# AsyncFlow-Sim/AsyncFlow

Measured on NVIDIA H100. Metric: simulated request-completions/sec, higher is better.
Workload: dtype f64

## Files before the change

asyncflow_b200/_capi.py:

```python

from __future__ import annotations

import ctypes as C
from pathlib import Path

AF_ABI_VERSION = 1
AF_HIST_BINS = 4096
AF_HIST_SUB_BITS = 7
AF_HIST_MIN_EXP = -20

DIST = {"poisson": 0, "normal": 1, "log_normal": 2, "exponential": 3, "uniform": 4}
TARGET_CLIENT, TARGET_LB, TARGET_SERVER = 0, 1, 2
STEP_CPU, STEP_IO = 0, 1
LB_NONE, LB_ROUND_ROBIN, LB_LEAST_CONNECTIONS = -1, 0, 1
METRIC_BITS = {"ready_queue_len": 1, "event_loop_io_sleep": 2, "ram_in_use": 4,
               "edge_concurrent_connection": 8}
FIELDS = {
    "users_mean": 0, "users_sigma": 1, "rate_per_user": 2, "edge_mean": 3, "edge_sigma": 4,
    "edge_dropout": 5, "server_cpu_cores": 6, "server_ram_mb": 7, "step_duration": 8,
    "endpoint_ram": 9, "spike_delta": 10,
}
FLAG_EVENT_OVERFLOW, FLAG_REQUEST_OVERFLOW, FLAG_TRACE_TRUNCATED, FLAG_NOWQ_OVERFLOW, FLAG_LB_EMPTY = 1, 2, 4, 8, 16
MODE_AUTO, MODE_WARP, MODE_LANE, MODE_TWO_PASS = 0, 1, 2, 3
SELFTEST_EDGE, SELFTEST_GEN_UNIFORM, SELFTEST_GEN_USERS, SELFTEST_ENDPOINT = 0, 1, 2, 3
MODES = {"auto": MODE_AUTO, "warp": MODE_WARP, "lane": MODE_LANE, "two_pass": MODE_TWO_PASS}


class AfEdge(C.Structure):
    _fields_ = [("mean", C.c_double), ("sigma", C.c_double), ("dropout", C.c_double),
                ("dist", C.c_int32), ("target_kind", C.c_int32), ("target_index", C.c_int32),
                ("reserved", C.c_int32)]


class AfServer(C.Structure):
    _fields_ = [("cpu_cores", C.c_int32), ("ram_mb", C.c_int32), ("out_edge", C.c_int32),
                ("endpoint_begin", C.c_int32), ("n_endpoints", C.c_int32), ("reserved", C.c_int32)]


class AfEndpoint(C.Structure):
    _fields_ = [("step_begin", C.c_int32), ("n_steps", C.c_int32), ("total_ram", C.c_int32),
                ("reserved", C.c_int32)]


class AfStep(C.Structure):
    _fields_ = [("duration", C.c_double), ("kind", C.c_int32), ("reserved", C.c_int32)]


class AfSpikeMark(C.Structure):
    _fields_ = [("fire_time", C.c_double), ("delta", C.c_double), ("edge", C.c_int32),
                ("reserved", C.c_int32)]


class AfOutageMark(C.Structure):
    _fields_ = [("fire_time", C.c_double), ("lb_edge", C.c_int32), ("down", C.c_int32)]


class AfScenario(C.Structure):
    _fields_ = [
        ("users_dist", C.c_int32), ("window_s", C.c_int32),
        ("users_mean", C.c_double), ("users_sigma", C.c_double), ("rate_per_user", C.c_double),
        ("horizon_s", C.c_int32), ("metrics_mask", C.c_uint32), ("sample_period", C.c_double),
        ("n_edges", C.c_int32), ("n_servers", C.c_int32), ("n_endpoints", C.c_int32),
        ("n_steps", C.c_int32), ("n_lb_edges", C.c_int32), ("lb_algo", C.c_int32),
        ("gen_edge", C.c_int32), ("client_edge", C.c_int32),
        ("n_spike_marks", C.c_int32), ("n_outage_marks", C.c_int32),
        ("edges", C.POINTER(AfEdge)), ("servers", C.POINTER(AfServer)),
        ("endpoints", C.POINTER(AfEndpoint)), ("steps", C.POINTER(AfStep)),
        ("lb_edges", C.POINTER(C.c_int32)), ("spike_marks", C.POINTER(AfSpikeMark)),
        ("outage_marks", C.POINTER(AfOutageMark)),
    ]


class AfSweepColumn(C.Structure):
    _fields_ = [("field", C.c_int32), ("index", C.c_int32)]


class AfSweep(C.Structure):
    _fields_ = [("n_columns", C.c_int32), ("reserved", C.c_int32), ("n_rows", C.c_uint64),
                ("columns", C.POINTER(AfSweepColumn)), ("values", C.POINTER(C.c_double))]


class AfOptions(C.Structure):
    _fields_ = [("event_capacity", C.c_int32), ("request_capacity", C.c_int32),
                ("warps_per_block", C.c_int32), ("blocks_per_sm", C.c_int32),
                ("collect_histogram", C.c_int32), ("collect_throughput", C.c_int32),
                ("trace_replicas", C.c_int32), ("trace_clock_capacity", C.c_int32)]


class AfReplicaStats(C.Structure):
    _fields_ = [("n_events", C.c_uint64), ("generated", C.c_uint32), ("completed", C.c_uint32),
                ("flags", C.c_uint32), ("n_ticks", C.c_uint32), ("peak_events", C.c_uint32),
                ("peak_requests", C.c_uint32), ("lat_sum", C.c_double), ("lat_sumsq", C.c_double),
                ("lat_min", C.c_double), ("lat_max", C.c_double), ("p50", C.c_double),
                ("p95", C.c_double), ("p99", C.c_double)]


import numpy as np

STATS_DTYPE = np.dtype([
    ("n_events", "<u8"), ("generated", "<u4"), ("completed", "<u4"), ("flags", "<u4"),
    ("n_ticks", "<u4"), ("peak_events", "<u4"), ("peak_requests", "<u4"),
    ("lat_sum", "<f8"), ("lat_sumsq", "<f8"), ("lat_min", "<f8"), ("lat_max", "<f8"),
    ("p50", "<f8"), ("p95", "<f8"), ("p99", "<f8"),
], align=True)
assert STATS_DTYPE.itemsize == C.sizeof(AfReplicaStats)


class AfRunPasses(C.Structure):
    _fields_ = [("lane_pass", C.c_int32), ("warp_pass", C.c_int32), ("lane_warps_per_sm", C.c_int32),
                ("lane_bytes", C.c_int32), ("lane_events_smem", C.c_int32), ("lane_requests_smem", C.c_int32),
                ("lane_replicas", C.c_uint64), ("warp_replicas", C.c_uint64)]


class EngineUnavailable(RuntimeError):
    """The CUDA engine cannot run here (library not built or no usable GPU)."""


LIB_PATH = Path(__file__).resolve().parent / "_lib" / "libasyncflow_b200.so"

EXPORTS = [
    "af_abi_version", "af_engine_create", "af_engine_destroy", "af_last_error",
    "af_engine_configure", "af_scenario_upload", "af_sweep_upload", "af_run", "af_sync",
    "af_last_run_ms", "af_launch_count", "af_fetch_stats", "af_fetch_edge_counts",
    "af_fetch_histograms", "af_fetch_throughput", "af_fetch_sampled", "af_fetch_trace_clocks",
    "af_fetch_trace_series", "af_reduce_histograms", "af_engine_set_mode", "af_last_run_passes",
    "af_selftest_rng",
]

_lib = None


def load() -> C.CDLL:
    global _lib
    if _lib is not None:
        return _lib
    import os
    path = Path(os.environ.get("ASYNCFLOW_B200_LIB", LIB_PATH))
    if not path.exists():
        msg = (f"{path} is missing: build it with `python -c 'import __graft_entry__ as g; "
               "g.build()'` (nvcc, sm_90a).  asyncflow_b200 has no CPU fallback.")
        raise EngineUnavailable(msg)
    lib = C.CDLL(str(path))
    vp, u64, i32 = C.c_void_p, C.c_uint64, C.c_int
    lib.af_abi_version.restype = i32
    lib.af_engine_create.argtypes = [i32, C.POINTER(vp)]
    lib.af_engine_destroy.argtypes = [vp]
    lib.af_engine_destroy.restype = None
    lib.af_last_error.argtypes = [vp]
    lib.af_last_error.restype = C.c_char_p
    lib.af_engine_configure.argtypes = [vp, C.POINTER(AfOptions)]
    lib.af_scenario_upload.argtypes = [vp, C.POINTER(AfScenario)]
    lib.af_sweep_upload.argtypes = [vp, C.POINTER(AfSweep), u64]
    lib.af_run.argtypes = [vp, u64, u64, u64]
    lib.af_sync.argtypes = [vp]
    lib.af_last_run_ms.argtypes = [vp, C.POINTER(C.c_float), C.POINTER(C.c_float)]
    lib.af_launch_count.argtypes = [vp]
    lib.af_launch_count.restype = u64
    lib.af_fetch_stats.argtypes = [vp, vp, u64]
    lib.af_fetch_edge_counts.argtypes = [vp, vp, vp, u64]
    lib.af_fetch_histograms.argtypes = [vp, vp, u64]
    lib.af_fetch_throughput.argtypes = [vp, vp, u64]
    lib.af_fetch_sampled.argtypes = [vp, vp, vp, u64]
    lib.af_fetch_trace_clocks.argtypes = [vp, u64, vp, u64, C.POINTER(u64)]
    lib.af_fetch_trace_series.argtypes = [vp, u64, vp, u64, C.POINTER(u64)]
    lib.af_reduce_histograms.argtypes = [vp, vp]
    lib.af_engine_set_mode.argtypes = [vp, i32]
    lib.af_last_run_passes.argtypes = [vp, C.POINTER(AfRunPasses)]
    lib.af_selftest_rng.argtypes = [vp, u64, u64, i32, i32, C.c_double, C.c_double, C.c_uint32, u64, vp, vp]
    for name in EXPORTS:
        fn = getattr(lib, name)
        if fn.restype is C.c_int and name not in ("af_abi_version",):
            fn.restype = i32
    if lib.af_abi_version() != AF_ABI_VERSION:
        msg = f"ABI mismatch: library {lib.af_abi_version()} != python {AF_ABI_VERSION}"
        raise EngineUnavailable(msg)
    _lib = lib
    return lib
```

asyncflow_b200/csrc/af_engine.cu:

```cuda
#include <cuda_runtime.h>
#include <stdio.h>
#include <stdlib.h>
#include <string.h>
#include <mutex>
#include <new>
#include <string>
#include <vector>

#include "af_host_common.h"
#include "af_lane_host.h"

#ifndef AF_LANE_DEFAULT_WARPS
#define AF_LANE_DEFAULT_WARPS 12
#endif

#ifndef AF_MIN_BLOCKS
#define AF_MIN_BLOCKS 8
#endif
#if AF_MIN_BLOCKS > 0
#define AF_LAUNCH_BOUNDS __launch_bounds__(128, AF_MIN_BLOCKS)
#else
#define AF_LAUNCH_BOUNDS
#endif

__global__ void AF_LAUNCH_BOUNDS af_sim_kernel() {
    extern __shared__ __align__(16) unsigned char af_smem[];
    const int warp = (int)(threadIdx.x >> 5);
    const int lane = (int)(threadIdx.x & 31u);
    unsigned char* ws = af_smem + (size_t)warp * (size_t)afc::c_L.warp_bytes;
    const uint64_t warp_slot = (uint64_t)blockIdx.x * (blockDim.x >> 5) + (uint64_t)warp;
    afc::State& W = *reinterpret_cast<afc::State*>(ws);
    afc::bind(W, ws, warp_slot);
    __syncwarp();
    for (;;) {
        unsigned long long r = 0;
        if (lane == 0) r = atomicAdd(afc::c_G.work_counter, 1ull);
        r = __shfl_sync(0xFFFFFFFFu, r, 0);
        if (afc::c_G.redo_list) {
            if (r >= (unsigned long long)*afc::c_G.redo_count) break;
            r = afc::c_G.redo_list[r];
        } else if (r >= afc::c_G.n_replicas) break;
        afc::run_replica(W, (uint64_t)r);
        __syncwarp();
    }
}

#ifndef AF_LANE_MAX_THREADS
#define AF_LANE_MAX_THREADS 384
#endif
__global__ void __launch_bounds__(AF_LANE_MAX_THREADS, 1) af_lane_kernel() {
    const afl::Cfg& C = afl::c_cfg;
    const uint32_t warp = threadIdx.x >> 5, lane = threadIdx.x & 31u;
    const uint32_t ws = warp * (uint32_t)C.warp_bytes;
    unsigned char* gs = C.gtier + ((uint64_t)blockIdx.x * (blockDim.x >> 5) + warp) * C.gwarp_bytes;
    afl::Mem m;
    m.s128 = ws + lane * 16u;
    m.s64 = ws + (uint32_t)C.n128 * (uint32_t)afl::STRIDE128 + lane * 8u;
    m.s32 = ws + (uint32_t)C.n128 * (uint32_t)afl::STRIDE128 + (uint32_t)C.n64 * (uint32_t)afl::STRIDE64 + lane * 4u;
    m.g128 = gs + lane * 16u;
    m.g64 = gs + (size_t)C.gn128 * afl::STRIDE128 + lane * 8u;
    m.g32 = gs + (size_t)C.gn128 * afl::STRIDE128 + (size_t)C.gn64 * afl::STRIDE64 + lane * 4u;
    afl::run_lane(m,
        [&]() -> uint64_t {
            const unsigned long long k = atomicAdd(C.work_counter, 1ull);
            return k < C.n_replicas ? (uint64_t)k : ~0ull;
        },
        [](bool alive) -> bool { return __any_sync(0xFFFFFFFFu, alive) != 0; });
}

__global__ void af_flagged_kernel(const AfReplicaStats* __restrict__ stats, uint64_t n, uint32_t mask,
                                  uint32_t* __restrict__ list, uint32_t* __restrict__ count) {
    const uint64_t i = (uint64_t)blockIdx.x * blockDim.x + threadIdx.x;
    if (i < n && (stats[i].flags & mask)) list[atomicAdd(count, 1u)] = (uint32_t)i;
}

__global__ void af_selftest_rng_kernel(uint64_t seed, uint64_t replica, int kind, int dist, double mean, double sigma,
                                       uint32_t hop, uint64_t n, double* __restrict__ a, double* __restrict__ b) {
    const uint64_t i = (uint64_t)blockIdx.x * blockDim.x + threadIdx.x;
    if (i >= n) return;
    if (kind == AF_SELFTEST_EDGE) {
        const afr::EdgeDraw d = afr::edge_draw(seed, replica, (uint32_t)i + 1u, hop, dist, mean, sigma, 0.0);
        a[i] = d.u; b[i] = d.transit;
    } else if (kind == AF_SELFTEST_GEN_UNIFORM) {
        afr::Src s = afr::make_gen(seed, replica, (uint32_t)i);
        double u = s.next53();
        a[i] = u;
        if (u < 1e-15) u = 1e-15;
        b[i] = -afr::af_log(1.0 - u);
    } else if (kind == AF_SELFTEST_GEN_USERS) {
        const afr::GenDraw g = afr::gen_users(seed, replica + i, 0u, dist, mean, sigma);
        a[i] = g.value; b[i] = (double)g.pos;
    } else {
        afr::Src src = afr::make_request(seed, replica, afr::P_SERVER, (uint32_t)i + 1u, hop);
        src.load(0);
        a[i] = (double)(uint32_t)(((uint64_t)src.w.x * (uint32_t)dist) >> 32); b[i] = 0.0;
    }
}

__device__ __forceinline__ double af_bin_value(int bin, uint64_t rank, uint64_t cum_before, uint32_t cnt) {
    const long long base = (long long)((1023 + AF_HIST_MIN_EXP) << AF_HIST_SUB_BITS);
    double lo = __longlong_as_double(((long long)bin + base) << (52 - AF_HIST_SUB_BITS));
    double hi = __longlong_as_double(((long long)bin + 1 + base) << (52 - AF_HIST_SUB_BITS));
    double frac = ((double)(rank - cum_before) + 0.5) / (double)cnt;
    return lo + frac * (hi - lo);
}

__global__ void af_percentile_kernel(const uint32_t* __restrict__ hist, AfReplicaStats* __restrict__ stats,
                                     uint64_t n_replicas) {
    const uint64_t warp = ((uint64_t)blockIdx.x * blockDim.x + threadIdx.x) >> 5;
    const int lane = (int)(threadIdx.x & 31u);
    if (warp >= n_replicas) return;
    const uint32_t* row = hist + warp * AF_HIST_BINS;
    const uint64_t n = stats[warp].completed;
    const double qs[3] = {50.0, 95.0, 99.0};
    uint64_t rank[6]; double frac[3]; double val[6];
#pragma unroll
    for (int i = 0; i < 3; ++i) {
        double pos = n ? qs[i] / 100.0 * (double)(n - 1) : 0.0;
        uint64_t lo = (uint64_t)floor(pos);
        frac[i] = pos - (double)lo;
        rank[2 * i] = lo;
        rank[2 * i + 1] = (lo + 1 < n) ? lo + 1 : lo;
        val[2 * i] = val[2 * i + 1] = 0.0;
    }
    uint64_t carry = 0;
    for (int base = 0; base < AF_HIST_BINS; base += 32) {
        uint32_t c = row[base + lane];
        uint32_t incl = c;
#pragma unroll
        for (int d = 1; d < 32; d <<= 1) {
            uint32_t up = __shfl_up_sync(0xFFFFFFFFu, incl, d);
            if (lane >= d) incl += up;
        }
        uint64_t before = carry + (incl - c);
#pragma unroll
        for (int i = 0; i < 6; ++i)
            if (c && rank[i] >= before && rank[i] < before + c) val[i] = af_bin_value(base + lane, rank[i], before, c);
        carry += __shfl_sync(0xFFFFFFFFu, incl, 31);
    }
#pragma unroll
    for (int i = 0; i < 6; ++i) {
        double v = val[i];
#pragma unroll
        for (int d = 16; d > 0; d >>= 1) v += __shfl_xor_sync(0xFFFFFFFFu, v, d);
        val[i] = v;
    }
    if (lane == 0) {
        const double nan = __longlong_as_double(0x7FF8000000000000ll);
        double p[3];
#pragma unroll
        for (int i = 0; i < 3; ++i)
            p[i] = n ? ((frac[i] == 0.0 || rank[2 * i + 1] == rank[2 * i]) ? val[2 * i]
                                                                            : val[2 * i] + frac[i] * (val[2 * i + 1] - val[2 * i]))
                     : nan;
        stats[warp].p50 = p[0]; stats[warp].p95 = p[1]; stats[warp].p99 = p[2];
    }
}


__global__ void af_hist_reduce_kernel(const uint32_t* __restrict__ hist, unsigned long long* __restrict__ total,
                                      uint64_t n_replicas, uint64_t rows_per_block) {
    uint64_t r0 = (uint64_t)blockIdx.x * rows_per_block;
    uint64_t r1 = r0 + rows_per_block < n_replicas ? r0 + rows_per_block : n_replicas;
    unsigned long long acc[AF_HIST_BINS / 256];
#pragma unroll
    for (int j = 0; j < AF_HIST_BINS / 256; ++j) acc[j] = 0;
    for (uint64_t r = r0; r < r1; ++r) {
        const uint32_t* row = hist + r * AF_HIST_BINS;
#pragma unroll
        for (int j = 0; j < AF_HIST_BINS / 256; ++j) acc[j] += row[j * 256 + threadIdx.x];
    }
#pragma unroll
    for (int j = 0; j < AF_HIST_BINS / 256; ++j)
        if (acc[j]) atomicAdd(&total[j * 256 + threadIdx.x], acc[j]);
}

namespace {

struct DevBuf {
    void* p = nullptr; size_t cap = 0;
    cudaError_t ensure(size_t bytes) {
        if (bytes <= cap) return cudaSuccess;
        if (p) cudaFree(p);
        p = nullptr; cap = 0;
        cudaError_t e = cudaMalloc(&p, bytes ? bytes : 1);
        if (e == cudaSuccess) cap = bytes;
        return e;
    }
    void release() { if (p) cudaFree(p); p = nullptr; cap = 0; }
};

thread_local std::string g_create_error;

constexpr int kMaxDevices = 64;
std::mutex g_const_mutex;
af_engine* g_const_owner[kMaxDevices] = {};

}

struct af_engine {
    int device = 0;
    int sm_count = 0;
    int max_smem_optin = 0;
    cudaStream_t stream = nullptr;
    cudaEvent_t ev_begin = nullptr, ev_sim = nullptr, ev_end = nullptr;
    std::string err;
    AfOptions opt{};
    bool have_scenario = false;
    AfScenario sc{};
    std::vector<AfEdge> h_edges; std::vector<AfServer> h_servers; std::vector<AfEndpoint> h_eps;
    std::vector<AfStep> h_steps; std::vector<int32_t> h_lb; std::vector<AfSpikeMark> h_spikes;
    std::vector<AfOutageMark> h_outages;
    DevBuf d_edges, d_servers, d_eps, d_steps, d_lb, d_spikes, d_outages;
    int32_t sweep_cols = 0; uint64_t sweep_rows = 0, sweep_first = 0;
    std::vector<AfSweepColumn> h_sweep_cols;
    std::vector<int32_t> h_sweep_alias;
    int32_t ev_need = 0;
    DevBuf d_sweep_cols, d_sweep_vals;
    int mode = AF_MODE_AUTO;
    aflh::Tables lt;
    DevBuf d_l_edges, d_l_servers, d_l_eps, d_l_steps, d_l_spikes, d_l_outages, d_l_lb, d_l_cols, d_gtier, d_redo_list, d_redo_count, d_counter2;
    afl::Cfg C_host{};
    bool last_lane = false, last_warp = false; int last_lane_warps = 0;
    DevBuf d_sp_evt, d_sp_evk, d_sp_rq, d_sp_nx;
    DevBuf d_stats, d_sent, d_dropped, d_hist, d_thr, d_ssum, d_smax, d_tclk, d_tser, d_tcnt, d_counter, d_htot;
    uint64_t last_n = 0; bool ran = false;
    afc::Layout L{};
    afc::Globals G_host{};
    uint64_t launches = 0;
    float ms_total = 0.f, ms_sim = 0.f; bool timing_valid = false;

    int fail(int code, const std::string& m) { err = m; return code; }
    int cuda_fail(cudaError_t e, const char* what) {
        err = std::string(what) + ": " + cudaGetErrorString(e);
        return AF_ERR_CUDA;
    }
};

#define AF_CUDA(e_, call, what) do { cudaError_t _c = (call); if (_c != cudaSuccess) return (e_)->cuda_fail(_c, what); } while (0)

template <class T>
static int upload_vec(af_engine* e, DevBuf& d, const std::vector<T>& h, const char* what) {
    AF_CUDA(e, d.ensure(h.size() * sizeof(T)), what);
    if (!h.empty()) AF_CUDA(e, cudaMemcpyAsync(d.p, h.data(), h.size() * sizeof(T), cudaMemcpyHostToDevice, e->stream), what);
    return AF_OK;
}

extern "C" {

int af_abi_version(void) { return AF_ABI_VERSION; }

const char* af_last_error(const af_engine* e) { return e ? e->err.c_str() : g_create_error.c_str(); }

int af_engine_create(int device, af_engine** out) {
    if (!out) { g_create_error = "out is NULL"; return AF_ERR_INVALID; }
    *out = nullptr;
    int n = 0;
    cudaError_t ce = cudaGetDeviceCount(&n);
    if (ce != cudaSuccess || n == 0) {
        g_create_error = std::string("no CUDA device: ") + (ce != cudaSuccess ? cudaGetErrorString(ce) : "count is 0")
                         + " (asyncflow_b200 has no CPU fallback)";
        return AF_ERR_CUDA;
    }
    if (device < 0 || device >= n) { g_create_error = "device index out of range"; return AF_ERR_INVALID; }
    cudaDeviceProp prop;
    if ((ce = cudaGetDeviceProperties(&prop, device)) != cudaSuccess) { g_create_error = cudaGetErrorString(ce); return AF_ERR_CUDA; }
    if (prop.major != 9 || prop.minor != 0) {
        char b[160]; snprintf(b, sizeof b, "device %d is sm_%d%d; this library carries sm_90a code only", device, prop.major, prop.minor);
        g_create_error = b; return AF_ERR_CUDA;
    }
    af_engine* e = new (std::nothrow) af_engine();
    if (!e) { g_create_error = "host allocation failed"; return AF_ERR_NOMEM; }
    e->device = device; e->sm_count = prop.multiProcessorCount; e->max_smem_optin = (int)prop.sharedMemPerBlockOptin;
    if ((ce = cudaSetDevice(device)) != cudaSuccess || (ce = cudaStreamCreateWithFlags(&e->stream, cudaStreamNonBlocking)) != cudaSuccess
        || (ce = cudaEventCreate(&e->ev_begin)) != cudaSuccess || (ce = cudaEventCreate(&e->ev_sim)) != cudaSuccess
        || (ce = cudaEventCreate(&e->ev_end)) != cudaSuccess) {
        g_create_error = cudaGetErrorString(ce); delete e; return AF_ERR_CUDA;
    }
    e->opt.collect_histogram = 1; e->opt.collect_throughput = 1;
    if (const char* m = getenv("ASYNCFLOW_B200_ENGINE")) {
        if (!strcmp(m, "warp")) e->mode = AF_MODE_WARP; else if (!strcmp(m, "lane")) e->mode = AF_MODE_LANE;
        else if (!strcmp(m, "two_pass")) e->mode = AF_MODE_TWO_PASS;
    }
    *out = e;
    return AF_OK;
}

void af_engine_destroy(af_engine* e) {
    if (!e) return;
    cudaSetDevice(e->device);
    cudaStreamSynchronize(e->stream);
    {
        std::lock_guard<std::mutex> lock(g_const_mutex);
        if (g_const_owner[e->device % kMaxDevices] == e) g_const_owner[e->device % kMaxDevices] = nullptr;
    }
    DevBuf* bufs[] = {&e->d_l_edges, &e->d_l_servers, &e->d_l_eps, &e->d_l_steps, &e->d_l_spikes, &e->d_l_outages, &e->d_l_lb, &e->d_l_cols,
                      &e->d_gtier, &e->d_redo_list, &e->d_redo_count, &e->d_counter2,
                      &e->d_edges, &e->d_servers, &e->d_eps, &e->d_steps, &e->d_lb, &e->d_spikes, &e->d_outages,
                      &e->d_sweep_cols, &e->d_sweep_vals, &e->d_sp_evt, &e->d_sp_evk, &e->d_sp_rq, &e->d_sp_nx,
                      &e->d_stats, &e->d_sent, &e->d_dropped, &e->d_hist, &e->d_thr, &e->d_ssum, &e->d_smax,
                      &e->d_tclk, &e->d_tser, &e->d_tcnt, &e->d_counter, &e->d_htot};
    for (DevBuf* b : bufs) b->release();
    cudaEventDestroy(e->ev_begin); cudaEventDestroy(e->ev_sim); cudaEventDestroy(e->ev_end);
    cudaStreamDestroy(e->stream);
    delete e;
}

int af_engine_configure(af_engine* e, const AfOptions* opt) {
    if (!e || !opt) return AF_ERR_INVALID;
    if (opt->event_capacity < 0 || opt->request_capacity < 0 || opt->warps_per_block < 0 || opt->warps_per_block > 32 || opt->blocks_per_sm < 0
        || opt->trace_replicas < 0 || opt->trace_clock_capacity < 0)
        return e->fail(AF_ERR_INVALID, "AfOptions: negative or out-of-range field");
    e->opt = *opt;
    return AF_OK;
}

int af_scenario_upload(af_engine* e, const AfScenario* s) {
    if (!e || !s) return AF_ERR_INVALID;
    std::string why;
    if (!afh::validate(*s, why)) return e->fail(AF_ERR_INVALID, "scenario: " + why);
    AF_CUDA(e, cudaSetDevice(e->device), "cudaSetDevice");
    AF_CUDA(e, cudaStreamSynchronize(e->stream), "sync before upload");
    e->sc = *s;
    e->h_edges.assign(s->edges, s->edges + s->n_edges);
    e->h_servers.assign(s->servers, s->servers + s->n_servers);
    e->h_eps.assign(s->endpoints, s->endpoints + s->n_endpoints);
    e->h_steps.assign(s->steps, s->steps + s->n_steps);
    e->h_lb.assign(s->lb_edges, s->lb_edges + s->n_lb_edges);
    e->h_spikes.assign(s->spike_marks, s->spike_marks + s->n_spike_marks);
    e->h_outages.assign(s->outage_marks, s->outage_marks + s->n_outage_marks);
    int rc;
    if ((rc = upload_vec(e, e->d_edges, e->h_edges, "edges"))) return rc;
    if ((rc = upload_vec(e, e->d_servers, e->h_servers, "servers"))) return rc;
    if ((rc = upload_vec(e, e->d_eps, e->h_eps, "endpoints"))) return rc;
    if ((rc = upload_vec(e, e->d_steps, e->h_steps, "steps"))) return rc;
    if ((rc = upload_vec(e, e->d_lb, e->h_lb, "lb_edges"))) return rc;
    if ((rc = upload_vec(e, e->d_spikes, e->h_spikes, "spike_marks"))) return rc;
    if ((rc = upload_vec(e, e->d_outages, e->h_outages, "outage_marks"))) return rc;
    AF_CUDA(e, cudaStreamSynchronize(e->stream), "scenario upload");
    e->sc.edges = e->h_edges.data(); e->sc.servers = e->h_servers.data(); e->sc.endpoints = e->h_eps.data();
    e->sc.steps = e->h_steps.data(); e->sc.lb_edges = e->h_lb.data(); e->sc.spike_marks = e->h_spikes.data();
    e->sc.outage_marks = e->h_outages.data();
    e->have_scenario = true;
    e->sweep_cols = 0; e->sweep_rows = 0; e->h_sweep_cols.clear();
    e->ev_need = aflh::pending_events_estimate(e->sc, nullptr);
    e->ran = false;
    return AF_OK;
}

int af_sweep_upload(af_engine* e, const AfSweep* sw, uint64_t first_replica) {
    if (!e) return AF_ERR_INVALID;
    if (!e->have_scenario) return e->fail(AF_ERR_STATE, "af_sweep_upload before af_scenario_upload");
    AF_CUDA(e, cudaSetDevice(e->device), "cudaSetDevice");
    AF_CUDA(e, cudaStreamSynchronize(e->stream), "sync before sweep upload");
    if (!sw || sw->n_columns == 0 || sw->n_rows == 0) { e->sweep_cols = 0; e->sweep_rows = 0; e->h_sweep_cols.clear(); e->ev_need = aflh::pending_events_estimate(e->sc, nullptr); return AF_OK; }
    if (!sw->columns || !sw->values) return e->fail(AF_ERR_INVALID, "sweep: null columns/values");
    const AfScenario& s = e->sc;
    for (int c = 0; c < sw->n_columns; ++c) {
        int f = sw->columns[c].field, i = sw->columns[c].index, lim = 1;
        switch (f) {
        case AF_FIELD_USERS_MEAN: case AF_FIELD_USERS_SIGMA: case AF_FIELD_RATE_PER_USER: lim = 1; break;
        case AF_FIELD_EDGE_MEAN: case AF_FIELD_EDGE_SIGMA: case AF_FIELD_EDGE_DROPOUT: lim = s.n_edges; break;
        case AF_FIELD_SERVER_CPU_CORES: case AF_FIELD_SERVER_RAM_MB: lim = s.n_servers; break;
        case AF_FIELD_STEP_DURATION: lim = s.n_steps; break;
        case AF_FIELD_ENDPOINT_RAM: lim = s.n_endpoints; break;
        case AF_FIELD_SPIKE_DELTA: lim = s.n_spike_marks; break;
        default: return e->fail(AF_ERR_INVALID, "sweep: unknown field id");
        }
        if (i < 0 || i >= lim) return e->fail(AF_ERR_INVALID, "sweep: column index out of range");
    }
    for (uint64_t r = 0; r < sw->n_rows; ++r)
        for (int c = 0; c < sw->n_columns; ++c) {
            const double v = sw->values[r * (uint64_t)sw->n_columns + (uint64_t)c];
            bool ok = v == v && v - v == 0.0;
            switch (sw->columns[c].field) {
            case AF_FIELD_EDGE_DROPOUT: ok = ok && v >= 0.0 && v <= 1.0; break;
            case AF_FIELD_SERVER_CPU_CORES: case AF_FIELD_SERVER_RAM_MB: ok = ok && v >= 1.0 && v <= 2147483647.0; break;
            case AF_FIELD_ENDPOINT_RAM: ok = ok && v >= 0.0 && v <= 2147483647.0; break;
            case AF_FIELD_EDGE_MEAN: ok = ok && (v >= 0.0 || s.edges[sw->columns[c].index].dist == AF_DIST_LOG_NORMAL || s.edges[sw->columns[c].index].dist == AF_DIST_NORMAL); break;
            case AF_FIELD_USERS_SIGMA: ok = ok && v >= 0.0 && s.users_dist == AF_DIST_NORMAL; break;
            default: ok = ok && v >= 0.0; break;
            }
            if (!ok) {
                char b[200]; snprintf(b, sizeof b, "sweep: row %llu column %d (field %d, index %d): value %g out of range",
                                      (unsigned long long)r, c, sw->columns[c].field, sw->columns[c].index, v);
                return e->fail(AF_ERR_INVALID, b);
            }
        }
    e->h_sweep_cols.assign(sw->columns, sw->columns + sw->n_columns);
    e->h_sweep_alias = aflh::column_aliases(sw->values, sw->n_rows, sw->n_columns);
    e->ev_need = aflh::pending_events_estimate(e->sc, sw);
    size_t cb = (size_t)sw->n_columns * sizeof(AfSweepColumn), vb = (size_t)sw->n_columns * sw->n_rows * sizeof(double);
    AF_CUDA(e, e->d_sweep_cols.ensure(cb), "sweep columns");
    AF_CUDA(e, e->d_sweep_vals.ensure(vb), "sweep values");
    AF_CUDA(e, cudaMemcpyAsync(e->d_sweep_cols.p, sw->columns, cb, cudaMemcpyHostToDevice, e->stream), "sweep columns H2D");
    AF_CUDA(e, cudaMemcpyAsync(e->d_sweep_vals.p, sw->values, vb, cudaMemcpyHostToDevice, e->stream), "sweep values H2D");
    AF_CUDA(e, cudaStreamSynchronize(e->stream), "sweep upload");
    e->sweep_cols = sw->n_columns; e->sweep_rows = sw->n_rows; e->sweep_first = first_replica;
    return AF_OK;
}

static int32_t lane_budget(const af_engine* e, int warps) {
    int32_t b = (int32_t)((e->max_smem_optin / (warps * 32)) & ~3);
    if (const char* cap = getenv("ASYNCFLOW_B200_LANE_BYTES")) { const int32_t c = atoi(cap) & ~3; if (c > 0 && c < b) b = c; }
    return b;
}

int af_run(af_engine* e, uint64_t seed, uint64_t begin, uint64_t end) {
    if (!e) return AF_ERR_INVALID;
    if (!e->have_scenario) return e->fail(AF_ERR_STATE, "af_run before af_scenario_upload");
    if (end <= begin) return e->fail(AF_ERR_INVALID, "af_run: empty replica range");
    if (end - begin > 0xFFFFFFFFull) return e->fail(AF_ERR_INVALID, "af_run: more than 2^32 replicas in one call");
    AF_CUDA(e, cudaSetDevice(e->device), "cudaSetDevice");
    const uint64_t n = end - begin;
    int rc;

    bool lane = e->mode != AF_MODE_WARP;
    afl::Cfg& C = e->C_host;
    int lane_warps = 0;
    if (lane) {
        std::string why;
        const bool all_rows = e->sweep_cols > 0 && begin >= e->sweep_first && end - e->sweep_first <= e->sweep_rows;
        if (!aflh::build_tables(e->sc, e->h_sweep_cols.data(), e->sweep_cols, all_rows ? e->h_sweep_alias.data() : nullptr, e->lt, why)) {
            if (e->mode == AF_MODE_LANE) return e->fail(AF_ERR_INVALID, why);
            lane = false;
        }
    }
    AfOptions o = e->opt;
    if (lane) {
        if (e->mode == AF_MODE_AUTO || e->mode == AF_MODE_TWO_PASS) {
            if (o.event_capacity <= 0 || o.event_capacity > aflh::LANE_EVENT_CAPACITY) o.event_capacity = aflh::LANE_EVENT_CAPACITY;
            if (o.request_capacity <= 0 || o.request_capacity > aflh::LANE_REQUEST_CAPACITY) o.request_capacity = aflh::LANE_REQUEST_CAPACITY;
        }
        lane_warps = e->opt.warps_per_block > 0 ? e->opt.warps_per_block : AF_LANE_DEFAULT_WARPS;
        if (lane_warps > AF_LANE_MAX_THREADS / 32) lane_warps = AF_LANE_MAX_THREADS / 32;
        while (lane_warps > 1 && lane_budget(e, lane_warps) < aflh::min_lane_bytes(e->sc, e->lt) + 128)
            lane_warps -= lane_warps > 8 ? 4 : (lane_warps > 4 ? 2 : 1);
        if (e->mode == AF_MODE_AUTO && lane_warps < 4) lane = false;
        if (e->mode == AF_MODE_AUTO && n < 3ull * (uint64_t)e->sm_count * 32ull) lane = false;
        if (lane && e->opt.warps_per_block <= 0) {
            const uint64_t per_warp = (uint64_t)e->sm_count * 32ull;
            const uint64_t waves = (n + per_warp * (uint64_t)lane_warps - 1) / (per_warp * (uint64_t)lane_warps);
            int w = (int)((n + waves * per_warp - 1) / (waves * per_warp));
            if (w < 4) w = 4;
            if (w < lane_warps) lane_warps = w;
        }
    }
    if (lane) {
        memset(&C, 0, sizeof C);
        if (!aflh::make_cfg(e->sc, o, e->lt, lane_budget(e, lane_warps), afh::trace_tick_capacity(e->sc), 32, C, getenv("ASYNCFLOW_B200_EVEN_SPLIT") ? 0 : e->ev_need,
                            getenv("ASYNCFLOW_B200_RQ_MIN") ? atoi(getenv("ASYNCFLOW_B200_RQ_MIN")) : 2)) {
            if (e->mode == AF_MODE_LANE) return e->fail(AF_ERR_INVALID, "scenario tables do not fit a lane's shared memory (thread-per-replica engine)");
            lane = false;
        }
    }
    const bool warp = e->mode != AF_MODE_LANE;
    const bool redo = lane && warp;

    afc::Layout& L = e->L;
    memset(&L, 0, sizeof L);
    afh::make_layout(e->sc, e->opt, e->sweep_cols, L);

    int wpb = 4; size_t smem = 0; uint64_t grid = 0, warp_slots = 0;
    if (warp) {
        if (!lane && e->opt.warps_per_block > 0 && e->opt.warps_per_block < 4) wpb = e->opt.warps_per_block;
        smem = (size_t)wpb * (size_t)L.warp_bytes;
        while (wpb > 1 && smem > (size_t)e->max_smem_optin) { --wpb; smem = (size_t)wpb * (size_t)L.warp_bytes; }
        if (smem > (size_t)e->max_smem_optin)
            return e->fail(AF_ERR_INVALID, "scenario tables do not fit in shared memory (one warp needs more than the 227 KB opt-in limit)");
        AF_CUDA(e, cudaFuncSetAttribute(af_sim_kernel, cudaFuncAttributeMaxDynamicSharedMemorySize, (int)smem), "smem attribute");
        int bps = 0;
        AF_CUDA(e, cudaOccupancyMaxActiveBlocksPerMultiprocessor(&bps, af_sim_kernel, wpb * 32, smem), "occupancy");
        if (bps < 1) return e->fail(AF_ERR_CUDA, "kernel cannot be resident (occupancy 0)");
        if (e->opt.blocks_per_sm > 0 && e->opt.blocks_per_sm < bps) bps = e->opt.blocks_per_sm;
        grid = (uint64_t)e->sm_count * (uint64_t)bps;
        const uint64_t need_blocks = (n + wpb - 1) / wpb;
        if (grid > need_blocks) grid = need_blocks;
        warp_slots = grid * wpb;
    }
    uint64_t lgrid = 0; size_t lsmem = 0;
    if (lane) {
        lsmem = (size_t)lane_warps * (size_t)C.warp_bytes;
        AF_CUDA(e, cudaFuncSetAttribute(af_lane_kernel, cudaFuncAttributeMaxDynamicSharedMemorySize, (int)lsmem), "smem attribute");
        lgrid = (uint64_t)e->sm_count;
        const uint64_t need = (n + (uint64_t)lane_warps * 32 - 1) / ((uint64_t)lane_warps * 32);
        if (lgrid > need) lgrid = need;
    }

    if (warp) {
        const uint64_t ev_sp = (uint64_t)(L.ev_total - L.ev_smem), rq_sp = (uint64_t)(L.rq_total - L.rq_smem);
        AF_CUDA(e, e->d_sp_evt.ensure(warp_slots * ev_sp * 8 + 8), "spill events");
        AF_CUDA(e, e->d_sp_evk.ensure(warp_slots * ev_sp * 8 + 8), "spill events");
        AF_CUDA(e, e->d_sp_rq.ensure(warp_slots * rq_sp * 16 + 16), "spill requests");
        AF_CUDA(e, e->d_sp_nx.ensure(warp_slots * rq_sp * 4 + 4), "spill requests");
    }
    if (lane) {
        AF_CUDA(e, e->d_gtier.ensure(lgrid * (uint64_t)lane_warps * C.gwarp_bytes + 256), "lane global tiers");
        if ((rc = upload_vec(e, e->d_l_edges, e->lt.edges, "lane tables"))) return rc;
        if ((rc = upload_vec(e, e->d_l_servers, e->lt.servers, "lane tables"))) return rc;
        if ((rc = upload_vec(e, e->d_l_eps, e->lt.endpoints, "lane tables"))) return rc;
        if ((rc = upload_vec(e, e->d_l_steps, e->lt.steps, "lane tables"))) return rc;
        if ((rc = upload_vec(e, e->d_l_spikes, e->lt.spikes, "lane tables"))) return rc;
        if ((rc = upload_vec(e, e->d_l_outages, e->lt.outages, "lane tables"))) return rc;
        if ((rc = upload_vec(e, e->d_l_lb, e->lt.lb, "lane tables"))) return rc;
        if ((rc = upload_vec(e, e->d_l_cols, e->lt.cols, "lane tables"))) return rc;
        AF_CUDA(e, e->d_counter2.ensure(8), "work counter");
        AF_CUDA(e, e->d_redo_list.ensure(n * 4), "flagged-replica list");
        AF_CUDA(e, e->d_redo_count.ensure(4), "flagged-replica count");
    }
    const uint64_t ntr = (uint64_t)(L.trace_replicas < 0 ? 0 : L.trace_replicas) < n ? (uint64_t)L.trace_replicas : n;
    L.trace_replicas = (int32_t)ntr; C.trace_replicas = (int32_t)ntr;
    AF_CUDA(e, e->d_stats.ensure(n * sizeof(AfReplicaStats)), "stats");
    AF_CUDA(e, e->d_sent.ensure(n * L.n_edges * 4), "edge counts");
    AF_CUDA(e, e->d_dropped.ensure(n * L.n_edges * 4), "edge counts");
    AF_CUDA(e, e->d_ssum.ensure(n * L.n_series * 8), "sampled sums");
    AF_CUDA(e, e->d_smax.ensure(n * L.n_series * 4), "sampled maxima");
    AF_CUDA(e, e->d_counter.ensure(8), "work counter");
    if (L.collect_hist) AF_CUDA(e, e->d_hist.ensure(n * AF_HIST_BINS * 4), "histograms");
    if (L.collect_thr) AF_CUDA(e, e->d_thr.ensure(n * (uint64_t)L.horizon_s * 4), "throughput");
    if (ntr) {
        AF_CUDA(e, e->d_tclk.ensure(ntr * (uint64_t)L.trace_clock_cap * 16 + 16), "trace clocks");
        AF_CUDA(e, e->d_tser.ensure(ntr * (uint64_t)L.n_series * (uint64_t)L.trace_tick_cap * 4 + 4), "trace series");
    }
    AF_CUDA(e, e->d_tcnt.ensure((ntr ? ntr : 1) * 8), "trace counts");

    afc::Globals G;
    memset(&G, 0, sizeof G);
    G.edges = (const AfEdge*)e->d_edges.p; G.servers = (const AfServer*)e->d_servers.p;
    G.endpoints = (const AfEndpoint*)e->d_eps.p; G.steps = (const AfStep*)e->d_steps.p;
    G.lb_edges = (const int32_t*)e->d_lb.p; G.spikes = (const AfSpikeMark*)e->d_spikes.p;
    G.outages = (const AfOutageMark*)e->d_outages.p;
    G.sweep_cols = (const AfSweepColumn*)e->d_sweep_cols.p; G.sweep_vals = (const double*)e->d_sweep_vals.p;
    G.sweep_first = e->sweep_first; G.sweep_rows = e->sweep_cols ? e->sweep_rows : 0;
    G.spill_ev_time = (double*)e->d_sp_evt.p; G.spill_ev_key = (uint64_t*)e->d_sp_evk.p;
    G.spill_rq_rec = (afc::ReqRec*)e->d_sp_rq.p; G.spill_rq_next = (uint32_t*)e->d_sp_nx.p;
    G.stats = (AfReplicaStats*)e->d_stats.p; G.edge_sent = (uint32_t*)e->d_sent.p; G.edge_dropped = (uint32_t*)e->d_dropped.p;
    G.hist = (uint32_t*)e->d_hist.p; G.thr = (uint32_t*)e->d_thr.p;
    G.samp_sum = (uint64_t*)e->d_ssum.p; G.samp_max = (uint32_t*)e->d_smax.p;
    G.trace_clocks = (double*)e->d_tclk.p; G.trace_series = (uint32_t*)e->d_tser.p; G.trace_counts = (uint32_t*)e->d_tcnt.p;
    G.work_counter = (unsigned long long*)e->d_counter.p;
    G.redo_list = redo ? (const uint32_t*)e->d_redo_list.p : nullptr;
    G.redo_count = redo ? (const uint32_t*)e->d_redo_count.p : nullptr;
    G.seed = seed; G.replica_begin = begin; G.n_replicas = n;
    if (lane) {
        C.edges = (const afl::EdgeP*)e->d_l_edges.p; C.servers = (const afl::ServerP*)e->d_l_servers.p;
        C.endpoints = (const afl::EndpointP*)e->d_l_eps.p; C.steps = (const afl::StepP*)e->d_l_steps.p;
        C.spikes = (const afl::SpikeP*)e->d_l_spikes.p; C.outages = (const afl::OutageP*)e->d_l_outages.p;
        C.lb_edges = (const int32_t*)e->d_l_lb.p; C.cols = (const afl::ColP*)e->d_l_cols.p;
        C.sweep_vals = G.sweep_vals; C.sweep_first = G.sweep_first; C.sweep_rows = G.sweep_rows;
        C.gtier = (unsigned char*)e->d_gtier.p;
        C.stats = G.stats; C.edge_sent = G.edge_sent; C.edge_dropped = G.edge_dropped; C.hist = G.hist; C.thr = G.thr;
        C.samp_sum = G.samp_sum; C.samp_max = G.samp_max; C.trace_clocks = G.trace_clocks; C.trace_series = G.trace_series;
        C.trace_counts = G.trace_counts;
        C.work_counter = (unsigned long long*)e->d_counter2.p;
        C.seed = seed; C.replica_begin = begin; C.n_replicas = n;
    }

    std::lock_guard<std::mutex> lock(g_const_mutex);
    {
        af_engine*& owner = g_const_owner[e->device % kMaxDevices];
        if (owner && owner != e) AF_CUDA(e, cudaStreamSynchronize(owner->stream), "waiting for the device's previous engine");
        owner = e;
    }
    AF_CUDA(e, cudaEventRecord(e->ev_begin, e->stream), "event");
    AF_CUDA(e, cudaMemsetAsync(e->d_counter.p, 0, 8, e->stream), "memset");
    if (L.collect_hist) AF_CUDA(e, cudaMemsetAsync(e->d_hist.p, 0, n * AF_HIST_BINS * 4, e->stream), "memset hist");
    if (L.collect_thr) AF_CUDA(e, cudaMemsetAsync(e->d_thr.p, 0, n * (uint64_t)L.horizon_s * 4, e->stream), "memset thr");
    if (lane) {
        AF_CUDA(e, cudaMemsetAsync(e->d_counter2.p, 0, 8, e->stream), "memset");
        AF_CUDA(e, cudaMemsetAsync(e->d_redo_count.p, 0, 4, e->stream), "memset");
        AF_CUDA(e, cudaMemcpyToSymbolAsync(afl::c_cfg, &C, sizeof C, 0, cudaMemcpyHostToDevice, e->stream), "lane config -> constant memory");
        af_lane_kernel<<<(unsigned)lgrid, lane_warps * 32, lsmem, e->stream>>>();
        AF_CUDA(e, cudaGetLastError(), "af_lane_kernel launch");
        e->launches += 1;
        if (redo) {
            af_flagged_kernel<<<(unsigned)((n + 255) / 256), 256, 0, e->stream>>>((const AfReplicaStats*)e->d_stats.p, n,
                AF_FLAG_EVENT_OVERFLOW | AF_FLAG_REQUEST_OVERFLOW | AF_FLAG_NOWQ_OVERFLOW, (uint32_t*)e->d_redo_list.p, (uint32_t*)e->d_redo_count.p);
            AF_CUDA(e, cudaGetLastError(), "af_flagged_kernel launch");
            e->launches += 1;
        }
    }
    if (warp) {
        AF_CUDA(e, cudaMemcpyToSymbolAsync(afc::c_L, &L, sizeof L, 0, cudaMemcpyHostToDevice, e->stream), "layout -> constant memory");
        e->G_host = G;
        AF_CUDA(e, cudaMemcpyToSymbolAsync(afc::c_G, &e->G_host, sizeof G, 0, cudaMemcpyHostToDevice, e->stream), "globals -> constant memory");
        af_sim_kernel<<<(unsigned)grid, wpb * 32, smem, e->stream>>>();
        AF_CUDA(e, cudaGetLastError(), "af_sim_kernel launch");
        e->launches += 1;
    }
    AF_CUDA(e, cudaEventRecord(e->ev_sim, e->stream), "event");
    if (L.collect_hist) {
        unsigned blocks = (unsigned)((n * 32 + 255) / 256);
        af_percentile_kernel<<<blocks, 256, 0, e->stream>>>((const uint32_t*)e->d_hist.p, (AfReplicaStats*)e->d_stats.p, n);
        AF_CUDA(e, cudaGetLastError(), "af_percentile_kernel launch");
        e->launches += 1;
    }
    AF_CUDA(e, cudaEventRecord(e->ev_end, e->stream), "event");
    e->last_n = n; e->ran = true; e->timing_valid = false;
    e->last_lane = lane; e->last_warp = warp; e->last_lane_warps = lane_warps;
    return AF_OK;
}

int af_selftest_rng(af_engine* e, uint64_t seed, uint64_t replica, int kind, int dist, double mean, double sigma,
                    uint32_t hop, uint64_t n, double* out_a, double* out_b) {
    if (!e || !out_a || !out_b || n == 0) return AF_ERR_INVALID;
    if (kind < AF_SELFTEST_EDGE || kind > AF_SELFTEST_ENDPOINT) return e->fail(AF_ERR_INVALID, "af_selftest_rng: unknown kind");
    AF_CUDA(e, cudaSetDevice(e->device), "cudaSetDevice");
    DevBuf da, db;
    cudaError_t ce;
    if ((ce = da.ensure(n * 8)) != cudaSuccess || (ce = db.ensure(n * 8)) != cudaSuccess) { da.release(); db.release(); return e->cuda_fail(ce, "selftest buffers"); }
    af_selftest_rng_kernel<<<(unsigned)((n + 255) / 256), 256, 0, e->stream>>>(seed, replica, kind, dist, mean, sigma, hop, n, (double*)da.p, (double*)db.p);
    e->launches += 1;
    ce = cudaGetLastError();
    if (ce == cudaSuccess) ce = cudaMemcpyAsync(out_a, da.p, n * 8, cudaMemcpyDeviceToHost, e->stream);
    if (ce == cudaSuccess) ce = cudaMemcpyAsync(out_b, db.p, n * 8, cudaMemcpyDeviceToHost, e->stream);
    if (ce == cudaSuccess) ce = cudaStreamSynchronize(e->stream);
    da.release(); db.release();
    if (ce != cudaSuccess) return e->cuda_fail(ce, "af_selftest_rng");
    return AF_OK;
}

int af_engine_set_mode(af_engine* e, int mode) {
    if (!e) return AF_ERR_INVALID;
    if (mode != AF_MODE_AUTO && mode != AF_MODE_WARP && mode != AF_MODE_LANE && mode != AF_MODE_TWO_PASS) return e->fail(AF_ERR_INVALID, "af_engine_set_mode: unknown mode");
    e->mode = mode;
    return AF_OK;
}

int af_last_run_passes(af_engine* e, AfRunPasses* out) {
    if (!e || !out) return AF_ERR_INVALID;
    if (!e->ran) return e->fail(AF_ERR_STATE, "no run yet");
    int rc = af_sync(e);
    if (rc) return rc;
    memset(out, 0, sizeof *out);
    out->lane_pass = e->last_lane ? 1 : 0; out->warp_pass = e->last_warp ? 1 : 0;
    out->lane_warps_per_sm = e->last_lane_warps;
    out->lane_bytes = e->last_lane ? e->C_host.warp_bytes / 32 : 0;
    out->lane_events_smem = e->last_lane ? e->C_host.ev_s : 0; out->lane_requests_smem = e->last_lane ? e->C_host.rq_s : 0;
    out->lane_replicas = e->last_lane ? e->last_n : 0;
    out->warp_replicas = e->last_warp ? e->last_n : 0;
    if (e->last_lane && e->last_warp) {
        uint32_t c = 0;
        AF_CUDA(e, cudaMemcpyAsync(&c, e->d_redo_count.p, 4, cudaMemcpyDeviceToHost, e->stream), "flagged count D2H");
        AF_CUDA(e, cudaStreamSynchronize(e->stream), "flagged count D2H");
        out->warp_replicas = c;
    }
    return AF_OK;
}

int af_sync(af_engine* e) {
    if (!e) return AF_ERR_INVALID;
    AF_CUDA(e, cudaSetDevice(e->device), "cudaSetDevice");
    AF_CUDA(e, cudaStreamSynchronize(e->stream), "af_sync");
    if (e->ran && !e->timing_valid) {
        float a = 0.f, b = 0.f;
        if (cudaEventElapsedTime(&a, e->ev_begin, e->ev_end) == cudaSuccess
            && cudaEventElapsedTime(&b, e->ev_begin, e->ev_sim) == cudaSuccess) {
            e->ms_total = a; e->ms_sim = b; e->timing_valid = true;
        }
    }
    return AF_OK;
}

int af_last_run_ms(af_engine* e, float* ms_total, float* ms_sim) {
    if (!e) return AF_ERR_INVALID;
    if (!e->ran) return e->fail(AF_ERR_STATE, "no run yet");
    int rc = af_sync(e);
    if (rc) return rc;
    if (ms_total) *ms_total = e->ms_total;
    if (ms_sim) *ms_sim = e->ms_sim;
    return AF_OK;
}

uint64_t af_launch_count(const af_engine* e) { return e ? e->launches : 0; }

static int fetch(af_engine* e, void* dst, const DevBuf& src, size_t bytes, uint64_t n, const char* what) {
    if (!e || !dst) return AF_ERR_INVALID;
    if (!e->ran) return e->fail(AF_ERR_STATE, "fetch before af_run");
    if (n != e->last_n) return e->fail(AF_ERR_INVALID, "fetch: n differs from the last run's replica count");
    AF_CUDA(e, cudaSetDevice(e->device), "cudaSetDevice");
    AF_CUDA(e, cudaMemcpyAsync(dst, src.p, bytes, cudaMemcpyDeviceToHost, e->stream), what);
    return af_sync(e);
}

int af_fetch_stats(af_engine* e, AfReplicaStats* out, uint64_t n) {
    return fetch(e, out, e->d_stats, n * sizeof(AfReplicaStats), n, "stats D2H");
}
int af_fetch_edge_counts(af_engine* e, uint32_t* sent, uint32_t* dropped, uint64_t n) {
    int rc = fetch(e, sent, e->d_sent, n * e->L.n_edges * 4, n, "edge sent D2H");
    if (rc) return rc;
    return fetch(e, dropped, e->d_dropped, n * e->L.n_edges * 4, n, "edge dropped D2H");
}
int af_fetch_histograms(af_engine* e, uint32_t* out, uint64_t n) {
    if (e && e->ran && !e->L.collect_hist) return e->fail(AF_ERR_STATE, "histograms were not collected");
    return fetch(e, out, e->d_hist, n * AF_HIST_BINS * 4, n, "hist D2H");
}
int af_fetch_throughput(af_engine* e, uint32_t* out, uint64_t n) {
    if (e && e->ran && !e->L.collect_thr) return e->fail(AF_ERR_STATE, "throughput was not collected");
    return fetch(e, out, e->d_thr, n * (uint64_t)e->L.horizon_s * 4, n, "throughput D2H");
}
int af_fetch_sampled(af_engine* e, uint64_t* sums, uint32_t* maxima, uint64_t n) {
    int rc = fetch(e, sums, e->d_ssum, n * e->L.n_series * 8, n, "sampled sums D2H");
    if (rc) return rc;
    return fetch(e, maxima, e->d_smax, n * e->L.n_series * 4, n, "sampled maxima D2H");
}

int af_reduce_histograms(af_engine* e, uint64_t* out_bins) {
    if (!e || !out_bins) return AF_ERR_INVALID;
    if (!e->ran) return e->fail(AF_ERR_STATE, "reduce before af_run");
    if (!e->L.collect_hist) return e->fail(AF_ERR_STATE, "histograms were not collected");
    AF_CUDA(e, cudaSetDevice(e->device), "cudaSetDevice");
    AF_CUDA(e, e->d_htot.ensure(AF_HIST_BINS * 8), "histogram total");
    AF_CUDA(e, cudaMemsetAsync(e->d_htot.p, 0, AF_HIST_BINS * 8, e->stream), "memset");
    const uint64_t n = e->last_n;
    uint64_t blocks = (uint64_t)e->sm_count * 8;
    if (blocks > n) blocks = n;
    uint64_t rows = (n + blocks - 1) / blocks;
    blocks = (n + rows - 1) / rows;
    af_hist_reduce_kernel<<<(unsigned)blocks, 256, 0, e->stream>>>((const uint32_t*)e->d_hist.p,
                                                                  (unsigned long long*)e->d_htot.p, n, rows);
    AF_CUDA(e, cudaGetLastError(), "af_hist_reduce_kernel launch");
    e->launches += 1;
    AF_CUDA(e, cudaMemcpyAsync(out_bins, e->d_htot.p, AF_HIST_BINS * 8, cudaMemcpyDeviceToHost, e->stream), "hist total D2H");
    AF_CUDA(e, cudaStreamSynchronize(e->stream), "af_reduce_histograms");
    return AF_OK;
}

int af_fetch_trace_clocks(af_engine* e, uint64_t local, double* out, uint64_t cap_pairs, uint64_t* n_pairs) {
    if (!e || !out || !n_pairs) return AF_ERR_INVALID;
    if (!e->ran) return e->fail(AF_ERR_STATE, "fetch before af_run");
    if (local >= (uint64_t)e->L.trace_replicas) return e->fail(AF_ERR_INVALID, "replica was not traced");
    AF_CUDA(e, cudaSetDevice(e->device), "cudaSetDevice");
    uint32_t cnt[2];
    AF_CUDA(e, cudaMemcpyAsync(cnt, (uint32_t*)e->d_tcnt.p + local * 2, 8, cudaMemcpyDeviceToHost, e->stream), "trace counts");
    AF_CUDA(e, cudaStreamSynchronize(e->stream), "trace counts");
    uint64_t n = cnt[0];
    if (n > (uint64_t)e->L.trace_clock_cap) n = (uint64_t)e->L.trace_clock_cap;
    if (n > cap_pairs) n = cap_pairs;
    *n_pairs = n;
    if (n) AF_CUDA(e, cudaMemcpyAsync(out, (double*)e->d_tclk.p + local * (uint64_t)e->L.trace_clock_cap * 2, n * 16,
                                      cudaMemcpyDeviceToHost, e->stream), "trace clocks");
    return af_sync(e);
}

int af_fetch_trace_series(af_engine* e, uint64_t local, uint32_t* out, uint64_t cap_ticks, uint64_t* n_ticks) {
    if (!e || !out || !n_ticks) return AF_ERR_INVALID;
    if (!e->ran) return e->fail(AF_ERR_STATE, "fetch before af_run");
    if (local >= (uint64_t)e->L.trace_replicas) return e->fail(AF_ERR_INVALID, "replica was not traced");
    AF_CUDA(e, cudaSetDevice(e->device), "cudaSetDevice");
    uint32_t cnt[2];
    AF_CUDA(e, cudaMemcpyAsync(cnt, (uint32_t*)e->d_tcnt.p + local * 2, 8, cudaMemcpyDeviceToHost, e->stream), "trace counts");
    AF_CUDA(e, cudaStreamSynchronize(e->stream), "trace counts");
    uint64_t n = cnt[1];
    if (n > (uint64_t)e->L.trace_tick_cap) n = (uint64_t)e->L.trace_tick_cap;
    if (n > cap_ticks) n = cap_ticks;
    *n_ticks = n;
    const uint32_t* base = (const uint32_t*)e->d_tser.p + local * (uint64_t)e->L.n_series * (uint64_t)e->L.trace_tick_cap;
    if (n) AF_CUDA(e, cudaMemcpy2DAsync(out, cap_ticks * 4, base, (size_t)e->L.trace_tick_cap * 4, n * 4, (size_t)e->L.n_series,
                                        cudaMemcpyDeviceToHost, e->stream), "trace series");
    return af_sync(e);
}

}
```

asyncflow_b200/csrc/af_lane.cuh:

```cuda
#pragma once
#include "af_rng.cuh"
#include "../../include/asyncflow_b200.h"

#if defined(__CUDA_ARCH__)
#define AFL_DEVICE 1
#else
#define AFL_DEVICE 0
#endif

#if defined(__CUDACC__)
#define AFL_IN __host__ __device__ __forceinline__
#else
#define AFL_IN static inline
#endif

#define AFL_LIKELY(x) __builtin_expect(!!(x), 1)
#define AFL_UNLIKELY(x) __builtin_expect(!!(x), 0)

#if defined(AF_TRACE_HOST) && !AFL_DEVICE
#include <stdio.h>
#define AFL_TRACE(...) fprintf(stderr, __VA_ARGS__)
#else
#define AFL_TRACE(...) ((void)0)
#endif

namespace afl {

#if AFL_DEVICE
constexpr int LANES = 32;
#else
constexpr int LANES = 1;
#endif
constexpr int STRIDE128 = LANES * 16, STRIDE64 = LANES * 8, STRIDE32 = LANES * 4;

constexpr uint32_t NIL = 0xFFFFFFFFu;
constexpr uint64_t INF_BITS = 0x7FF0000000000000ull;

enum : uint32_t { K_ARRIVAL = 0, K_DELIVER = 1, K_STEP_END = 2, K_SPIKE = 3, K_OUTAGE = 4 };
constexpr uint32_t SLOT_BITS = 20, AUX_BITS = 9;
constexpr uint32_t SLOT_MASK = (1u << SLOT_BITS) - 1, AUX_MASK = (1u << AUX_BITS) - 1;
AFL_IN uint32_t mk_payload(uint32_t kind, uint32_t aux, uint32_t slot) { return (kind << 29) | (aux << SLOT_BITS) | slot; }

constexpr uint32_t PK_CORE = 1u << 28, PK_IO = 1u << 29, PK_WAIT = 1u << 30;
AFL_IN uint32_t pk_hops(uint32_t p) { return p & 0xFFu; }
AFL_IN uint32_t pk_step(uint32_t p) { return (p >> 8) & 0xFFu; }
AFL_IN uint32_t pk_ep(uint32_t p) { return (p >> 16) & 0xFFFu; }

enum : uint32_t { I_PUT = 0, I_GOT = 1, I_CLIENT_LOOP = 2, I_RAM_OK = 3, I_CPU_OK = 4, I_CPU_PUT = 5, I_RAM_PUT = 6 };
constexpr uint32_t NODE_CLIENT = 0, NODE_LB = 1, NODE_SERVER0 = 2;
constexpr int32_t NQ_TOTAL = 128;

struct alignas(16) EdgeP { double mean, sigma, dropout; uint32_t meta; int16_t c_mean, c_sigma, c_drop, pad; uint32_t pad2[2]; };
struct alignas(16) ServerP { int32_t cpu_cores, ram_mb; uint32_t out_edge, ep_begin, n_ep; int32_t c_cores, c_ram, pad; };
struct alignas(16) EndpointP { uint32_t step_begin, n_steps, total_ram; int32_t c_ram; };
struct alignas(16) StepP { double dur; uint32_t kind; int32_t c_dur; };
struct alignas(16) SpikeP { double fire, delta; uint32_t edge; int32_t c_delta; uint32_t pad[2]; };
struct alignas(16) OutageP { double fire; int32_t lb_edge, down; };
struct ColP { int32_t field, index, slot, pad; double base; };

enum : int32_t { SV_CPU_FREE = 0, SV_RAM_FREE, SV_READY_Q, SV_IO_Q, SV_RAM_IN_USE, SV_WORDS };
enum : int32_t { SQ_RAMQ_HEAD = 0, SQ_RAMQ_TAIL, SQ_CPUQ_HEAD, SQ_CPUQ_TAIL, SQ_RAMQ_NEED, SQ_WORDS };
enum : int32_t { IB_HEAD = 0, IB_TAIL, IB_PENDING, IB_WORDS };

struct Cfg {
    int32_t n_edges, n_servers, n_endpoints, n_steps, n_lb_edges, lb_algo;
    int32_t gen_edge, client_edge, n_spike, n_outage;
    int32_t users_dist, window_s, horizon_s;
    uint32_t metrics_mask;
    double users_mean, users_sigma, rate_per_user, sample_period;
    int32_t n_series, n_sweep_cols, n_row;
    int32_t collect_hist, collect_thr, trace_replicas, trace_clock_cap, trace_tick_cap;
    int32_t redo;
    int32_t ev_s, ev_total, rq_s, rq_total, nq_s;
    int32_t o128_ev, o128_rq, n128;
    int32_t o64_nq, o64_spike, o64_row, n64;
    int32_t o32_next, o32_conn, o32_srv, o32_lb, o32_dirty, n_dirty, n32;
    int32_t warp_bytes;
    int32_t gi_ev, gi_rq, gn128;
    int32_t gi_nq, gi_acc, gn64;
    int32_t gi_next, g32_cold, gi_smax, gi_sent, gn32;
    int32_t c_srvq, c_inbox, c_drop;
    uint64_t gwarp_bytes;
    const EdgeP* edges; const ServerP* servers; const EndpointP* endpoints; const StepP* steps;
    const SpikeP* spikes; const OutageP* outages; const int32_t* lb_edges; const ColP* cols;
    const double* sweep_vals; uint64_t sweep_first, sweep_rows;
    unsigned char* gtier;
    AfReplicaStats* stats; uint32_t* edge_sent; uint32_t* edge_dropped;
    uint32_t* hist; uint32_t* thr; uint64_t* samp_sum; uint32_t* samp_max;
    double* trace_clocks; uint32_t* trace_series; uint32_t* trace_counts;
    unsigned long long* work_counter;
    const uint32_t* redo_list; const uint32_t* redo_count;
    uint64_t seed, replica_begin, n_replicas;
};

#if defined(__CUDACC__)
__constant__ Cfg c_cfg;
#endif
#if AFL_DEVICE
#define AFL_C c_cfg
#else
static Cfg h_cfg;
#define AFL_C h_cfg
#endif

template <class T> AFL_IN T ro(const T* p) {
#if AFL_DEVICE
    static_assert(sizeof(T) % 16 == 0, "16-byte records");
    T v;
    const uint4* s = reinterpret_cast<const uint4*>(p);
    uint4* d = reinterpret_cast<uint4*>(&v);
#pragma unroll
    for (int i = 0; i < (int)(sizeof(T) / 16); ++i) d[i] = __ldg(s + i);
    return v;
#else
    return *p;
#endif
}

struct Mem {
    uint32_t s128, s64, s32;
    unsigned char* g128; unsigned char* g64; unsigned char* g32;
};
#if AFL_DEVICE
AFL_IN uint32_t sm_ld32(uint32_t a) { uint32_t v; asm volatile("ld.shared.u32 %0, [%1];" : "=r"(v) : "r"(a)); return v; }
AFL_IN void sm_st32(uint32_t a, uint32_t v) { asm volatile("st.shared.u32 [%0], %1;" :: "r"(a), "r"(v)); }
AFL_IN uint64_t sm_ld64(uint32_t a) { uint64_t v; asm volatile("ld.shared.u64 %0, [%1];" : "=l"(v) : "r"(a)); return v; }
AFL_IN void sm_st64(uint32_t a, uint64_t v) { asm volatile("st.shared.u64 [%0], %1;" :: "r"(a), "l"(v)); }
AFL_IN void sm_ld128(uint32_t a, uint64_t& x, uint64_t& y) { asm volatile("ld.shared.v2.u64 {%0, %1}, [%2];" : "=l"(x), "=l"(y) : "r"(a)); }
AFL_IN void sm_st128(uint32_t a, uint64_t x, uint64_t y) { asm volatile("st.shared.v2.u64 [%0], {%1, %2};" :: "r"(a), "l"(x), "l"(y)); }
AFL_IN void gl_ld128(const unsigned char* p, uint64_t& x, uint64_t& y) { const ulonglong2 v = *reinterpret_cast<const ulonglong2*>(p); x = v.x; y = v.y; }
AFL_IN void gl_st128(unsigned char* p, uint64_t x, uint64_t y) { *reinterpret_cast<ulonglong2*>(p) = make_ulonglong2(x, y); }
#else
static unsigned char* afl_smem_host = nullptr;
AFL_IN uint32_t sm_ld32(uint32_t a) { uint32_t v; memcpy(&v, afl_smem_host + a, 4); return v; }
AFL_IN void sm_st32(uint32_t a, uint32_t v) { memcpy(afl_smem_host + a, &v, 4); }
AFL_IN uint64_t sm_ld64(uint32_t a) { uint64_t v; memcpy(&v, afl_smem_host + a, 8); return v; }
AFL_IN void sm_st64(uint32_t a, uint64_t v) { memcpy(afl_smem_host + a, &v, 8); }
AFL_IN void sm_ld128(uint32_t a, uint64_t& x, uint64_t& y) { memcpy(&x, afl_smem_host + a, 8); memcpy(&y, afl_smem_host + a + 8, 8); }
AFL_IN void sm_st128(uint32_t a, uint64_t x, uint64_t y) { memcpy(afl_smem_host + a, &x, 8); memcpy(afl_smem_host + a + 8, &y, 8); }
AFL_IN void gl_ld128(const unsigned char* p, uint64_t& x, uint64_t& y) { memcpy(&x, p, 8); memcpy(&y, p + 8, 8); }
AFL_IN void gl_st128(unsigned char* p, uint64_t x, uint64_t y) { memcpy(p, &x, 8); memcpy(p + 8, &y, 8); }
#endif
AFL_IN uint32_t a128(const Mem& m, int32_t elem) { return m.s128 + (uint32_t)elem * (uint32_t)STRIDE128; }
AFL_IN uint32_t a64(const Mem& m, int32_t elem) { return m.s64 + (uint32_t)elem * (uint32_t)STRIDE64; }
AFL_IN uint32_t a32(const Mem& m, int32_t word) { return m.s32 + (uint32_t)word * (uint32_t)STRIDE32; }
AFL_IN unsigned char* g128p(const Mem& m, int32_t elem) { return m.g128 + (uint64_t)(uint32_t)elem * (uint32_t)STRIDE128; }
AFL_IN uint64_t* g64p(const Mem& m, int32_t elem) { return reinterpret_cast<uint64_t*>(m.g64 + (uint64_t)(uint32_t)elem * (uint32_t)STRIDE64); }
AFL_IN uint32_t* g32p(const Mem& m, int32_t word) { return reinterpret_cast<uint32_t*>(m.g32 + (uint64_t)(uint32_t)word * (uint32_t)STRIDE32); }
AFL_IN uint64_t e64_ld(const Mem& m, int32_t elem) { return sm_ld64(a64(m, elem)); }
AFL_IN void e64_st(const Mem& m, int32_t elem, uint64_t v) { sm_st64(a64(m, elem), v); }
AFL_IN double f64_ld(const Mem& m, int32_t elem) { return afr::u2d(e64_ld(m, elem)); }
AFL_IN void f64_st(const Mem& m, int32_t elem, double v) { e64_st(m, elem, afr::d2u(v)); }
AFL_IN uint32_t w32_ld(const Mem& m, int32_t word) { return sm_ld32(a32(m, word)); }
AFL_IN void w32_st(const Mem& m, int32_t word, uint32_t v) { sm_st32(a32(m, word), v); }
AFL_IN int32_t i32_ld(const Mem& m, int32_t word) { return (int32_t)w32_ld(m, word); }
AFL_IN void i32_st(const Mem& m, int32_t word, int32_t v) { w32_st(m, word, (uint32_t)v); }
AFL_IN uint32_t c32_ld(const Mem& m, int32_t word) { return *g32p(m, AFL_C.g32_cold + word); }
AFL_IN void c32_st(const Mem& m, int32_t word, uint32_t v) { *g32p(m, AFL_C.g32_cold + word) = v; }
AFL_IN void ld_t128(const Mem& m, int32_t os, int32_t gi, int32_t idx, int32_t split, uint64_t& x, uint64_t& y) {
    if (AFL_LIKELY(idx < split)) sm_ld128(a128(m, os + idx), x, y); else gl_ld128(g128p(m, gi + idx), x, y);
}
AFL_IN void st_t128(const Mem& m, int32_t os, int32_t gi, int32_t idx, int32_t split, uint64_t x, uint64_t y) {
    if (AFL_LIKELY(idx < split)) sm_st128(a128(m, os + idx), x, y); else gl_st128(g128p(m, gi + idx), x, y);
}
AFL_IN uint64_t ld_t64(const Mem& m, int32_t os, int32_t gi, int32_t idx, int32_t split) {
    if (AFL_LIKELY(idx < split)) return sm_ld64(a64(m, os + idx));
    return *g64p(m, gi + idx);
}
AFL_IN void st_t64(const Mem& m, int32_t os, int32_t gi, int32_t idx, int32_t split, uint64_t v) {
    if (AFL_LIKELY(idx < split)) sm_st64(a64(m, os + idx), v); else *g64p(m, gi + idx) = v;
}
AFL_IN uint32_t ld_t32(const Mem& m, int32_t os, int32_t gi, int32_t idx, int32_t split) {
    if (AFL_LIKELY(idx < split)) return sm_ld32(a32(m, os + idx));
    return *g32p(m, gi + idx);
}
AFL_IN void st_t32(const Mem& m, int32_t os, int32_t gi, int32_t idx, int32_t split, uint32_t v) {
    if (AFL_LIKELY(idx < split)) sm_st32(a32(m, os + idx), v); else *g32p(m, gi + idx) = v;
}

struct St {
    uint64_t replica, local;
    double now, horizon;
    uint32_t seq; int32_t ev_n; uint32_t peak_ev;
    uint64_t arr_t; uint32_t arr_seq, arr_on;
    uint32_t nq_head, nq_tail, busy;
    uint32_t rq_free, rq_free_hi, rq_hw, rq_live, peak_rq;
    uint32_t n_waiting;
    double g_vnow, g_wend, g_lam;
    uint32_t g_pos, generated, g_done, need_arrival, arm_seq;
    double gap0, gap1; uint32_t gap_cnt;
    double users_mean, users_sigma, rate_per_user;
    int32_t lb_n, spike_cur, outage_cur;
    uint32_t tick_seq, n_ticks; double tick_time;
    uint32_t completed, flags, traced;
    uint64_t n_events;
    double lat_sum, lat_sumsq, lat_min, lat_max;
};

constexpr uint32_t STOP_FLAGS = AF_FLAG_EVENT_OVERFLOW | AF_FLAG_REQUEST_OVERFLOW | AF_FLAG_NOWQ_OVERFLOW | AF_FLAG_LB_EMPTY;

AFL_IN double row_val(const Mem& m, int32_t c) { return f64_ld(m, AFL_C.o64_row + c); }
AFL_IN uint32_t ep_total_ram(const Mem& m, uint32_t ep) {
    const EndpointP p = ro(AFL_C.endpoints + ep);
    return p.c_ram >= 0 ? (uint32_t)row_val(m, p.c_ram) : p.total_ram;
}

AFL_IN void rq_load(const Mem& m, uint32_t s, double& t0, uint32_t& rid, uint32_t& pack) {
    uint64_t a, b;
    ld_t128(m, AFL_C.o128_rq, AFL_C.gi_rq, (int32_t)s, AFL_C.rq_s, a, b);
    t0 = afr::u2d(a); rid = (uint32_t)b; pack = (uint32_t)(b >> 32);
}
AFL_IN void rq_store(const Mem& m, uint32_t s, double t0, uint32_t rid, uint32_t pack) {
    st_t128(m, AFL_C.o128_rq, AFL_C.gi_rq, (int32_t)s, AFL_C.rq_s, afr::d2u(t0), (uint64_t)rid | ((uint64_t)pack << 32));
}
AFL_IN uint32_t rq_pack(const Mem& m, uint32_t s) {
    if (AFL_LIKELY((int32_t)s < AFL_C.rq_s)) return sm_ld32(a128(m, AFL_C.o128_rq + (int32_t)s) + 12u);
    return *reinterpret_cast<const uint32_t*>(g128p(m, AFL_C.gi_rq + (int32_t)s) + 12);
}
AFL_IN void rq_pack_set(const Mem& m, uint32_t s, uint32_t v) {
    if (AFL_LIKELY((int32_t)s < AFL_C.rq_s)) sm_st32(a128(m, AFL_C.o128_rq + (int32_t)s) + 12u, v);
    else *reinterpret_cast<uint32_t*>(g128p(m, AFL_C.gi_rq + (int32_t)s) + 12) = v;
}
AFL_IN uint32_t rq_next(const Mem& m, uint32_t s) { return ld_t32(m, AFL_C.o32_next, AFL_C.gi_next, (int32_t)s, AFL_C.rq_s); }
AFL_IN void rq_next_set(const Mem& m, uint32_t s, uint32_t v) { st_t32(m, AFL_C.o32_next, AFL_C.gi_next, (int32_t)s, AFL_C.rq_s, v); }

#if AFL_DEVICE
__device__ __forceinline__ void red_add64(uint64_t* p, uint64_t v) { atomicAdd(reinterpret_cast<unsigned long long*>(p), (unsigned long long)v); }
__device__ __forceinline__ void red_add32(uint32_t* p, uint32_t v) { atomicAdd(p, v); }
__device__ __forceinline__ void red_max32(uint32_t* p, uint32_t v) { atomicMax(p, v); }
__device__ __forceinline__ uint64_t ld_cg64(const uint64_t* p) { return (uint64_t)__ldcg(reinterpret_cast<const unsigned long long*>(p)); }
__device__ __forceinline__ uint32_t ld_cg32(const uint32_t* p) { return __ldcg(p); }
#else
static inline void red_add64(uint64_t* p, uint64_t v) { *p += v; }
static inline void red_add32(uint32_t* p, uint32_t v) { *p += v; }
static inline void red_max32(uint32_t* p, uint32_t v) { if (v > *p) *p = v; }
static inline uint64_t ld_cg64(const uint64_t* p) { return *p; }
static inline uint32_t ld_cg32(const uint32_t* p) { return *p; }
#endif
AFL_IN uint32_t rq_alloc(St& W, const Mem& m) {
    uint32_t s;
    if (W.rq_free != NIL) { s = W.rq_free; W.rq_free = rq_next(m, s); }
    else if ((int32_t)W.rq_hw < AFL_C.rq_s) { s = W.rq_hw++; }
    else if (W.rq_free_hi != NIL) { s = W.rq_free_hi; W.rq_free_hi = rq_next(m, s); }
    else if ((int32_t)W.rq_hw < AFL_C.rq_total) { s = W.rq_hw++; }
    else { W.flags |= AF_FLAG_REQUEST_OVERFLOW; return NIL; }
    const uint32_t live = ++W.rq_live;
    if (live > W.peak_rq) W.peak_rq = live;
    return s;
}
AFL_IN void rq_release(St& W, const Mem& m, uint32_t s) {
    if ((int32_t)s < AFL_C.rq_s) { rq_next_set(m, s, W.rq_free); W.rq_free = s; }
    else { rq_next_set(m, s, W.rq_free_hi); W.rq_free_hi = s; }
    --W.rq_live;
}

#if defined(__CUDACC__)
#define AFL_COLD __host__ __device__ __noinline__
#else
#define AFL_COLD static __attribute__((noinline))
#endif
AFL_COLD void fifo_push(const Mem m, int32_t w_head, int32_t w_tail, uint32_t s) {
    rq_next_set(m, s, NIL);
    const uint32_t tail = c32_ld(m, w_tail);
    if (tail == NIL) c32_st(m, w_head, s); else rq_next_set(m, tail, s);
    c32_st(m, w_tail, s);
}
AFL_COLD uint32_t fifo_pop(const Mem m, int32_t w_head, int32_t w_tail) {
    const uint32_t s = c32_ld(m, w_head);
    const uint32_t h = rq_next(m, s);
    c32_st(m, w_head, h);
    if (h == NIL) c32_st(m, w_tail, NIL);
    return s;
}

AFL_IN void ev_get(const Mem& m, int32_t i, uint64_t& t, uint64_t& k) { ld_t128(m, AFL_C.o128_ev, AFL_C.gi_ev, i, AFL_C.ev_s, t, k); }
AFL_IN void ev_set(const Mem& m, int32_t i, uint64_t t, uint64_t k) { st_t128(m, AFL_C.o128_ev, AFL_C.gi_ev, i, AFL_C.ev_s, t, k); }
AFL_IN bool ev_less(uint64_t ta, uint64_t ka, uint64_t tb, uint64_t kb) {
    return ta < tb || (ta == tb && (uint32_t)(ka >> 32) < (uint32_t)(kb >> 32));
}
AFL_IN void heap_push(St& W, const Mem& m, uint64_t tb, uint64_t key) {
    int32_t i = W.ev_n;
    const int32_t pending = i + (int32_t)W.arr_on;
    if (AFL_UNLIKELY(pending >= AFL_C.ev_total)) { W.flags |= AF_FLAG_EVENT_OVERFLOW; return; }
    W.ev_n = i + 1;
    if ((uint32_t)(pending + 1) > W.peak_ev) W.peak_ev = (uint32_t)(pending + 1);
#pragma unroll 1
    while (i > 0) {
        const int32_t p = (i - 1) >> 2;
        uint64_t tp, kp;
        ev_get(m, p, tp, kp);
        if (!ev_less(tb, key, tp, kp)) break;
        ev_set(m, i, tp, kp);
        i = p;
    }
    ev_set(m, i, tb, key);
}
AFL_IN void heap_pop(St& W, const Mem& m) {
    const int32_t n = --W.ev_n;
    if (n == 0) return;
    uint64_t tl, kl;
    ev_get(m, n, tl, kl);
    const int32_t last = n - 1;
    int32_t i = 0;
#pragma unroll 1
    for (;;) {
        const int32_t c = 4 * i + 1;
        if (c >= n) break;
        const int32_t c1 = c + 1 < last ? c + 1 : last, c3 = c + 3 < last ? c + 3 : last;
        int32_t c2 = c + 2 < last ? c + 2 : last;
        uint64_t t0, k0, t1, k1, t2, k2, t3, k3;
        if (AFL_LIKELY(c3 < AFL_C.ev_s)) {
            sm_ld128(a128(m, AFL_C.o128_ev + c), t0, k0); sm_ld128(a128(m, AFL_C.o128_ev + c1), t1, k1);
            sm_ld128(a128(m, AFL_C.o128_ev + c2), t2, k2); sm_ld128(a128(m, AFL_C.o128_ev + c3), t3, k3);
        } else {
            ev_get(m, c, t0, k0); ev_get(m, c1, t1, k1); ev_get(m, c2, t2, k2); ev_get(m, c3, t3, k3);
        }
        int32_t b = c;
        if (ev_less(t1, k1, t0, k0)) { t0 = t1; k0 = k1; b = c1; }
        if (ev_less(t3, k3, t2, k2)) { t2 = t3; k2 = k3; c2 = c3; }
        if (ev_less(t2, k2, t0, k0)) { t0 = t2; k0 = k2; b = c2; }
        if (!ev_less(t0, k0, tl, kl)) break;
        ev_set(m, i, t0, k0);
        i = b;
    }
    ev_set(m, i, tl, kl);
}

AFL_IN uint64_t nq_ld(const Mem& m, uint32_t pos) {
    return ld_t64(m, AFL_C.o64_nq, AFL_C.gi_nq, (int32_t)(pos & (uint32_t)(NQ_TOTAL - 1)), AFL_C.nq_s);
}
AFL_IN bool can_fuse(const St& W) { return AFL_LIKELY(W.busy == 0); }
AFL_IN void nq_push(St& W, const Mem& m, uint32_t kind, uint32_t aux, uint32_t slot) {
    const uint32_t tail = W.nq_tail;
    if (tail - W.nq_head >= (uint32_t)NQ_TOTAL) { W.flags |= AF_FLAG_NOWQ_OVERFLOW; return; }
    st_t64(m, AFL_C.o64_nq, AFL_C.gi_nq, (int32_t)(tail & (uint32_t)(NQ_TOTAL - 1)), AFL_C.nq_s,
           ((uint64_t)(W.seq++) << 32) | mk_payload(kind, aux, slot));
    W.nq_tail = tail + 1;
    W.busy += 2u;
}
AFL_IN uint32_t nq_take(St& W, const Mem& m) {
    const uint32_t item = (uint32_t)nq_ld(m, W.nq_head);
    W.nq_head += 1;
    if (W.nq_head == W.nq_tail) { W.nq_head = 0; W.nq_tail = 0; }
    return item;
}

AFL_IN bool gen_next_gap(St& W, double& gap) {
    const double T = W.horizon;
    double vnow = W.g_vnow, wend = W.g_wend, lam = W.g_lam;
    uint32_t pos = W.g_pos;
    bool ok = false;
#pragma unroll 1
    for (;;) {
        if (!(vnow < T)) break;
        if (vnow >= wend) {
            wend = vnow + (double)AFL_C.window_s;
            afr::GenDraw d = afr::gen_users(AFL_C.seed, W.replica, pos, AFL_C.users_dist, W.users_mean, W.users_sigma);
            pos = d.pos;
            lam = d.value * W.rate_per_user;
        }
        if (lam <= 0.0) { vnow = wend; continue; }
        afr::Src s = afr::make_gen(AFL_C.seed, W.replica, pos);
        double u = s.next53();
        pos = s.pos;
        if (u < 1e-15) u = 1e-15;
        const double dt = afr::af_div(-afr::af_log(1.0 - u), lam);
        if (vnow + dt > T) break;
        if (vnow + dt >= wend) { vnow = wend; continue; }
        vnow += dt;
        gap = dt;
        ok = true;
        break;
    }
    W.g_vnow = vnow; W.g_wend = wend; W.g_lam = lam; W.g_pos = pos;
    return ok;
}

AFL_IN void gauge_touch(const St& W, const Mem& m, int32_t j, uint32_t v_old, int32_t delta) {
    red_add64(g64p(m, AFL_C.gi_acc + j), (uint64_t)(int64_t)delta * (uint64_t)W.n_ticks);
    const int32_t dw = AFL_C.o32_dirty + (j >> 5);
    const uint32_t d = w32_ld(m, dw), bit = 1u << (j & 31);
    if (!(d & bit)) {
        red_max32(g32p(m, AFL_C.gi_smax + j), v_old);
        w32_st(m, dw, d | bit);
    }
}
AFL_IN void conn_add(const St& W, const Mem& m, uint32_t edge, int32_t delta) {
    const int32_t pw = AFL_C.o32_conn + (int32_t)edge;
    const uint32_t v = w32_ld(m, pw);
    if (AFL_C.metrics_mask & AF_METRIC_EDGE_CONN) gauge_touch(W, m, 3 * AFL_C.n_servers + (int32_t)edge, v, delta);
    w32_st(m, pw, v + (uint32_t)delta);
}
AFL_IN int32_t ib_word(uint32_t node, int32_t f) { return AFL_C.c_inbox + (int32_t)node * IB_WORDS + f; }
AFL_IN int32_t sq_word(uint32_t sidx, int32_t f) { return AFL_C.c_srvq + (int32_t)sidx * SQ_WORDS + f; }
AFL_IN int32_t sv_word(uint32_t sidx, int32_t f) { return AFL_C.o32_srv + (int32_t)sidx * SV_WORDS + f; }
AFL_IN void srv_gauge_add(const St& W, const Mem& m, uint32_t sidx, int32_t field, int32_t delta) {
    const int32_t pw = sv_word(sidx, field);
    const int32_t v = i32_ld(m, pw);
    if ((AFL_C.metrics_mask & 7u) == 7u) gauge_touch(W, m, 3 * (int32_t)sidx + (field - SV_READY_Q), (uint32_t)v, delta);
    i32_st(m, pw, v + delta);
}
AFL_IN uint32_t gauge_value(const Mem& m, int32_t j) {
    const int32_t ns3 = 3 * AFL_C.n_servers;
    if (j < ns3) { const int32_t mt = j % 3; return w32_ld(m, sv_word((uint32_t)(j / 3), mt == 0 ? SV_READY_Q : (mt == 1 ? SV_IO_Q : SV_RAM_IN_USE))); }
    return w32_ld(m, AFL_C.o32_conn + (j - ns3));
}
AFL_IN bool gauge_on(int32_t j) {
    return j < 3 * AFL_C.n_servers ? (AFL_C.metrics_mask & 7u) == 7u
                                   : (AFL_C.metrics_mask & AF_METRIC_EDGE_CONN) != 0;
}
AFL_IN void take_ticks(St& W, const Mem& m, double t, uint32_t ev_seq) {
    double tick = W.tick_time;
    uint32_t tseq = W.tick_seq, nt = W.n_ticks, seq = W.seq;
    const double horizon = W.horizon;
#pragma unroll 1
    while ((tick < t || (tick == t && tseq < ev_seq)) && tick < horizon) {
        if (AFL_UNLIKELY(W.traced != 0) && (int32_t)nt < AFL_C.trace_tick_cap) {
#pragma unroll 1
            for (int32_t j = 0; j < AFL_C.n_series; ++j)
                if (gauge_on(j)) AFL_C.trace_series[(W.local * (uint64_t)AFL_C.n_series + (uint32_t)j) * (uint64_t)AFL_C.trace_tick_cap + nt] = gauge_value(m, j);
        }
        nt += 1;
        tseq = seq++;
        tick = tick + AFL_C.sample_period;
    }
    if (nt != W.n_ticks) {
#pragma unroll 1
        for (int32_t w = 0; w < AFL_C.n_dirty; ++w) w32_st(m, AFL_C.o32_dirty + w, 0u);
    }
    W.tick_time = tick; W.tick_seq = tseq; W.n_ticks = nt; W.seq = seq;
}

AFL_IN bool q_empty(const St& W, const Mem& m, int32_t head) { return AFL_LIKELY(W.n_waiting == 0) || c32_ld(m, head) == NIL; }
AFL_IN void consumer_get(St& W, const Mem& m, uint32_t node) {
    if (AFL_UNLIKELY(c32_ld(m, ib_word(node, IB_HEAD)) != NIL)) {
        const uint32_t it = fifo_pop(m, ib_word(node, IB_HEAD), ib_word(node, IB_TAIL));
        nq_push(W, m, I_GOT, node, it);
    } else c32_st(m, ib_word(node, IB_PENDING), 1);
}
AFL_IN bool cpu_walk(St& W, const Mem& m, uint32_t sidx, uint32_t watch) {
    bool hit = false;
#pragma unroll 1
    while (!q_empty(W, m, sq_word(sidx, SQ_CPUQ_HEAD)) && i32_ld(m, sv_word(sidx, SV_CPU_FREE)) > 0) {
        const uint32_t w = fifo_pop(m, sq_word(sidx, SQ_CPUQ_HEAD), sq_word(sidx, SQ_CPUQ_TAIL));
        W.n_waiting -= 1;
        i32_st(m, sv_word(sidx, SV_CPU_FREE), i32_ld(m, sv_word(sidx, SV_CPU_FREE)) - 1);
        hit = hit || w == watch;
        nq_push(W, m, I_CPU_OK, sidx, w);
    }
    return hit;
}
AFL_IN void ram_walk(St& W, const Mem& m, uint32_t sidx) {
#pragma unroll 1
    while (!q_empty(W, m, sq_word(sidx, SQ_RAMQ_HEAD))) {
        const uint32_t need = c32_ld(m, sq_word(sidx, SQ_RAMQ_NEED));
        if ((int32_t)need > i32_ld(m, sv_word(sidx, SV_RAM_FREE))) break;
        const uint32_t w = fifo_pop(m, sq_word(sidx, SQ_RAMQ_HEAD), sq_word(sidx, SQ_RAMQ_TAIL));
        W.n_waiting -= 1;
        const uint32_t h = c32_ld(m, sq_word(sidx, SQ_RAMQ_HEAD));
        if (h != NIL) c32_st(m, sq_word(sidx, SQ_RAMQ_NEED), ep_total_ram(m, pk_ep(rq_pack(m, h))));
        i32_st(m, sv_word(sidx, SV_RAM_FREE), i32_ld(m, sv_word(sidx, SV_RAM_FREE)) - (int32_t)need);
        nq_push(W, m, I_RAM_OK, sidx, w);
    }
}

AFL_IN bool on_spike(St& W, const Mem& m, double& next_fire) {
    int32_t cur = W.spike_cur;
    const double t = ro(AFL_C.spikes + cur).fire;
#pragma unroll 1
    while (cur < AFL_C.n_spike) {
        const SpikeP p = ro(AFL_C.spikes + cur);
        if (p.fire != t) break;
        double delta = p.delta;
        if (p.c_delta >= 0) { const double v = row_val(m, p.c_delta); delta = delta < 0.0 ? -v : v; }
        f64_st(m, AFL_C.o64_spike + (int32_t)p.edge, f64_ld(m, AFL_C.o64_spike + (int32_t)p.edge) + delta);
        ++cur;
    }
    W.spike_cur = cur;
    if (cur < AFL_C.n_spike) { next_fire = ro(AFL_C.spikes + cur).fire; return true; }
    return false;
}
AFL_IN bool on_outage(St& W, const Mem& m, double& next_fire) {
    int32_t cur = W.outage_cur;
    const double t = ro(AFL_C.outages + cur).fire;
    int32_t n = W.lb_n;
    const int32_t lb = AFL_C.o32_lb;
#pragma unroll 1
    while (cur < AFL_C.n_outage) {
        const OutageP p = ro(AFL_C.outages + cur);
        if (p.fire != t) break;
        ++cur;
        if (p.lb_edge < 0) continue;
        int32_t at = -1;
#pragma unroll 1
        for (int32_t i = 0; i < n; ++i) if (w32_ld(m, lb + i) == (uint32_t)p.lb_edge) { at = i; break; }
        if (at >= 0) {
#pragma unroll 1
            for (int32_t i = at + 1; i < n; ++i) w32_st(m, lb + i - 1, w32_ld(m, lb + i));
            --n;
        }
        if (!p.down) { w32_st(m, lb + n, (uint32_t)p.lb_edge); ++n; }
    }
    W.lb_n = n;
    W.outage_cur = cur;
    if (cur < AFL_C.n_outage) { next_fire = ro(AFL_C.outages + cur).fire; return true; }
    return false;
}

#if AFL_DEVICE
__device__ __forceinline__ void red_add(uint32_t* p, uint32_t v) { atomicAdd(p, v); }
#else
static inline void red_add(uint32_t* p, uint32_t v) { *p += v; }
#endif

AFL_IN void complete(St& W, const Mem& m, uint32_t slot, double t0) {
    const double now = W.now;
    const double lat = now - t0;
    const uint32_t done = ++W.completed;
    W.lat_sum += lat;
    W.lat_sumsq += lat * lat;
    if (lat < W.lat_min) W.lat_min = lat;
    if (lat > W.lat_max) W.lat_max = lat;
    const uint64_t local = W.local;
    if (AFL_C.collect_hist) {
        int32_t idx = (int32_t)(afr::d2u(lat) >> (52 - AF_HIST_SUB_BITS)) - ((1023 + AF_HIST_MIN_EXP) << AF_HIST_SUB_BITS);
        idx = idx < 0 ? 0 : (idx >= AF_HIST_BINS ? AF_HIST_BINS - 1 : idx);
        red_add(&AFL_C.hist[local * AF_HIST_BINS + (uint32_t)idx], 1u);
    }
    if (AFL_C.collect_thr) {
        int32_t b = (int32_t)ceil(now) - 1;
        b = b < 0 ? 0 : b;
        if (b < AFL_C.horizon_s) red_add(&AFL_C.thr[local * (uint64_t)AFL_C.horizon_s + (uint32_t)b], 1u);
    }
    if (AFL_UNLIKELY(W.traced != 0)) {
        if ((int32_t)(done - 1) < AFL_C.trace_clock_cap) {
            double* p = AFL_C.trace_clocks + (local * (uint64_t)AFL_C.trace_clock_cap + (done - 1)) * 2;
            p[0] = t0; p[1] = now;
        } else W.flags |= AF_FLAG_TRACE_TRUNCATED;
    }
    rq_release(W, m, slot);
}

AFL_IN void start_replica(St& W, const Mem& m, uint64_t local_index) {
    const Cfg& C = AFL_C;
    W.local = local_index;
    W.replica = C.replica_begin + local_index;
    W.now = 0.0; W.horizon = (double)C.horizon_s; W.seq = 0;
    W.ev_n = 0; W.peak_ev = 0; W.arr_t = 0; W.arr_seq = 0; W.arr_on = 0;
    W.nq_head = 0; W.nq_tail = 0; W.busy = 0;
    W.rq_free = NIL; W.rq_free_hi = NIL; W.rq_hw = 0; W.rq_live = 0; W.peak_rq = 0; W.n_waiting = 0;
    W.g_vnow = 0.0; W.g_wend = 0.0; W.g_lam = 0.0; W.g_pos = 0; W.generated = 0; W.g_done = 0;
    W.gap0 = 0.0; W.gap1 = 0.0; W.gap_cnt = 0;
    W.lb_n = C.n_lb_edges; W.spike_cur = 0; W.outage_cur = 0;
    W.n_ticks = 0; W.completed = 0; W.flags = 0; W.n_events = 0;
    W.lat_sum = 0.0; W.lat_sumsq = 0.0; W.lat_min = afr::u2d(INF_BITS); W.lat_max = 0.0;
    W.traced = (int64_t)local_index < (int64_t)C.trace_replicas ? 1u : 0u;
    W.users_mean = C.users_mean; W.users_sigma = C.users_sigma; W.rate_per_user = C.rate_per_user;
#pragma unroll 1
    for (int32_t i = 0; i < C.n_edges; ++i) {
        w32_st(m, C.o32_conn + i, 0); *g32p(m, C.gi_sent + i) = 0; c32_st(m, C.c_drop + i, 0);
        if (C.n_spike > 0) f64_st(m, C.o64_spike + i, 0.0);
    }
#pragma unroll 1
    for (int32_t i = 0; i < C.n_servers; ++i) {
        const ServerP p = ro(C.servers + i);
        i32_st(m, sv_word((uint32_t)i, SV_CPU_FREE), p.cpu_cores); i32_st(m, sv_word((uint32_t)i, SV_RAM_FREE), p.ram_mb);
        i32_st(m, sv_word((uint32_t)i, SV_READY_Q), 0); i32_st(m, sv_word((uint32_t)i, SV_IO_Q), 0); i32_st(m, sv_word((uint32_t)i, SV_RAM_IN_USE), 0);
        c32_st(m, sq_word((uint32_t)i, SQ_RAMQ_HEAD), NIL); c32_st(m, sq_word((uint32_t)i, SQ_RAMQ_TAIL), NIL);
        c32_st(m, sq_word((uint32_t)i, SQ_CPUQ_HEAD), NIL); c32_st(m, sq_word((uint32_t)i, SQ_CPUQ_TAIL), NIL);
        c32_st(m, sq_word((uint32_t)i, SQ_RAMQ_NEED), 0);
    }
#pragma unroll 1
    for (int32_t i = 0; i < C.n_servers + 2; ++i) {
        c32_st(m, ib_word((uint32_t)i, IB_HEAD), NIL); c32_st(m, ib_word((uint32_t)i, IB_TAIL), NIL); c32_st(m, ib_word((uint32_t)i, IB_PENDING), 1);
    }
#pragma unroll 1
    for (int32_t i = 0; i < C.n_lb_edges; ++i) w32_st(m, C.o32_lb + i, (uint32_t)C.lb_edges[i]);
#pragma unroll 1
    for (int32_t j = 0; j < C.n_series; ++j) { *g64p(m, C.gi_acc + j) = 0; *g32p(m, C.gi_smax + j) = 0; }
#pragma unroll 1
    for (int32_t w = 0; w < C.n_dirty; ++w) w32_st(m, C.o32_dirty + w, 0xFFFFFFFFu);
    const bool has_row = C.n_sweep_cols > 0 && W.replica >= C.sweep_first && W.replica - C.sweep_first < C.sweep_rows;
    const double* row = C.sweep_vals + (has_row ? (W.replica - C.sweep_first) * (uint64_t)C.n_sweep_cols : 0);
#pragma unroll 1
    for (int32_t c = 0; c < C.n_sweep_cols; ++c) {
        const ColP col = C.cols[c];
        const double v = has_row ? row[c] : col.base;
        if (col.slot >= 0) { f64_st(m, C.o64_row + col.slot, v); continue; }
        if (!has_row) continue;
        switch (col.field) {
        case AF_FIELD_USERS_MEAN: W.users_mean = v; break;
        case AF_FIELD_USERS_SIGMA: W.users_sigma = v; break;
        case AF_FIELD_RATE_PER_USER: W.rate_per_user = v; break;
        case AF_FIELD_SERVER_CPU_CORES: i32_st(m, sv_word((uint32_t)col.index, SV_CPU_FREE), (int32_t)v); break;
        case AF_FIELD_SERVER_RAM_MB: i32_st(m, sv_word((uint32_t)col.index, SV_RAM_FREE), (int32_t)v); break;
        default: break;
        }
    }
    if (C.redo) {
        if (C.collect_hist) for (int32_t b = 0; b < AF_HIST_BINS; ++b) C.hist[W.local * AF_HIST_BINS + (uint32_t)b] = 0;
        if (C.collect_thr) for (int32_t b = 0; b < C.horizon_s; ++b) C.thr[W.local * (uint64_t)C.horizon_s + (uint32_t)b] = 0;
    }
}

AFL_IN void write_back(St& W, const Mem& m) {
    const Cfg& C = AFL_C;
    const uint64_t local = W.local;
#pragma unroll 1
    for (int32_t i = 0; i < C.n_edges; ++i) {
        C.edge_sent[local * (uint64_t)C.n_edges + (uint32_t)i] = ld_cg32(g32p(m, C.gi_sent + i));
        C.edge_dropped[local * (uint64_t)C.n_edges + (uint32_t)i] = c32_ld(m, C.c_drop + i);
    }
#pragma unroll 1
    for (int32_t j = 0; j < C.n_series; ++j) {
        uint64_t sum = 0; uint32_t mx = 0;
        if (gauge_on(j)) {
            const uint32_t v = gauge_value(m, j);
            sum = (uint64_t)W.n_ticks * (uint64_t)v - ld_cg64(g64p(m, C.gi_acc + j));
            mx = ld_cg32(g32p(m, C.gi_smax + j));
            if (!((w32_ld(m, C.o32_dirty + (j >> 5)) >> (j & 31)) & 1u) && v > mx) mx = v;
        }
        C.samp_sum[local * (uint64_t)C.n_series + (uint32_t)j] = sum;
        C.samp_max[local * (uint64_t)C.n_series + (uint32_t)j] = mx;
    }
    AfReplicaStats st;
    st.n_events = W.n_events; st.generated = W.generated; st.completed = W.completed;
    st.flags = W.flags; st.n_ticks = W.n_ticks; st.peak_events = W.peak_ev; st.peak_requests = W.peak_rq;
    st.lat_sum = W.lat_sum; st.lat_sumsq = W.lat_sumsq;
    st.lat_min = W.completed ? W.lat_min : 0.0; st.lat_max = W.lat_max;
    st.p50 = st.p95 = st.p99 = afr::u2d(0x7FF8000000000000ull);
    C.stats[local] = st;
    if (W.traced) { C.trace_counts[local * 2] = W.completed; C.trace_counts[local * 2 + 1] = W.n_ticks; }
}

enum : uint32_t { A_NONE = 0, A_NODE, A_STEPS, A_SEND, A_TIMER };

#if AFL_DEVICE
#define AFL_SYNC() __syncwarp()
#else
#define AFL_SYNC() ((void)0)
#endif

template <class NextFn, class ConvFn>
AFL_IN void run_lane(const Mem& m, NextFn next_index, ConvFn converge) {
    const Cfg& C = AFL_C;
    St W;
    bool active = false, exhausted = false;
#pragma unroll 1
    for (;;) {
        if (!converge(active || !exhausted)) break;
        if (AFL_UNLIKELY(!active && !exhausted)) {
            const uint64_t r = next_index();
            if (r == ~0ull) exhausted = true;
            else {
                start_replica(W, m, r);
                if (C.n_spike > 0) {
                    double f = ro(C.spikes).fire;
                    bool arm = true;
                    if (f == 0.0) arm = on_spike(W, m, f);
                    if (arm && f < W.horizon) { if (f == W.now) W.busy |= 1u; heap_push(W, m, afr::d2u(f), ((uint64_t)(W.seq++) << 32) | mk_payload(K_SPIKE, 0, 0)); }
                }
                if (C.n_outage > 0) {
                    double f = ro(C.outages).fire;
                    bool arm = true;
                    if (f == 0.0) arm = on_outage(W, m, f);
                    if (arm && f < W.horizon) { if (f == W.now) W.busy |= 1u; heap_push(W, m, afr::d2u(f), ((uint64_t)(W.seq++) << 32) | mk_payload(K_OUTAGE, 0, 0)); }
                }
                W.arm_seq = W.seq++; W.need_arrival = 1;
                W.tick_seq = W.seq++;
                W.tick_time = 0.0 + C.sample_period;
                active = true;
            }
        }
        AFL_SYNC();
        const bool run = active;
        const bool dead = run && (W.flags & STOP_FLAGS) != 0;
        if (run && W.need_arrival && !dead) {
            W.need_arrival = 0;
            double gap = 0.0;
            bool have = false;
            if (W.gap_cnt) { gap = W.gap0; W.gap0 = W.gap1; W.gap_cnt -= 1u; have = true; }
            else if (!W.g_done && gen_next_gap(W, gap)) have = true;
            if (have) {
                const double t = W.now + gap;
                if (t < W.horizon) {
                    if (AFL_UNLIKELY(t == W.now)) W.busy |= 1u;
                    if (AFL_UNLIKELY(W.ev_n >= AFL_C.ev_total)) W.flags |= AF_FLAG_EVENT_OVERFLOW;
                    else {
                        W.arr_t = afr::d2u(t); W.arr_seq = W.arm_seq; W.arr_on = 1u;
                        if ((uint32_t)W.ev_n + 1u > W.peak_ev) W.peak_ev = (uint32_t)W.ev_n + 1u;
                    }
                }
            } else W.g_done = 1;
        }
        AFL_SYNC();
        uint32_t word = 0;
        bool is_item = false, finish = false, is_event = false;
        double t_ev = 0.0; uint32_t ev_seq = 0;
        if (run) {
            if (AFL_UNLIKELY(dead)) finish = true;
            else {
                const uint32_t busy = W.busy;
                const bool have_item = busy >= 2u;
                if (have_item && !(busy & 1u)) {
                    W.busy = busy - 2u;
                    word = nq_take(W, m);
                    is_item = true;
                } else {
                    const bool have_heap = W.ev_n > 0, have_ev = have_heap || W.arr_on != 0;
                    uint64_t tb = 0, key = 0;
                    if (have_heap) sm_ld128(a128(m, AFL_C.o128_ev), tb, key);
                    const uint64_t root_t = tb;
                    bool take_arr = false;
                    if (W.arr_on) {
                        const uint64_t ak = ((uint64_t)W.arr_seq << 32) | mk_payload(K_ARRIVAL, 0, 0);
                        if (!have_heap || ev_less(W.arr_t, ak, tb, key)) { tb = W.arr_t; key = ak; take_arr = true; }
                    }
                    if (have_item) {
                        const uint64_t front = nq_ld(m, W.nq_head);
                        const bool same_t = have_ev && tb == afr::d2u(W.now);
                        if (!(same_t && (uint32_t)(key >> 32) < (uint32_t)(front >> 32))) {
                            W.busy = (same_t ? busy : (busy & ~1u)) - 2u;
                            word = nq_take(W, m);
                            is_item = true;
                        }
                    } else if (!have_ev) finish = true;
                    if (!is_item && !finish) {
                        bool more;
                        if (take_arr) { W.arr_on = 0u; more = have_heap && root_t == tb; }
                        else { heap_pop(W, m); more = (W.ev_n > 0 && sm_ld64(a128(m, AFL_C.o128_ev)) == tb) || (W.arr_on && W.arr_t == tb); }
                        W.busy = (W.busy & ~1u) | (more ? 1u : 0u);
                        t_ev = afr::u2d(tb); ev_seq = (uint32_t)(key >> 32); word = (uint32_t)key;
                        is_event = true;
                    }
                }
            }
            if (finish) { t_ev = W.horizon; ev_seq = 0u; }
        }
        AFL_SYNC();
        if (run && !is_item) {
            const double tick = W.tick_time;
            if (tick < t_ev || (tick == t_ev && W.tick_seq < ev_seq)) take_ticks(W, m, t_ev, ev_seq);
        }
        if (AFL_UNLIKELY(finish)) { write_back(W, m); active = false; }
        AFL_SYNC();
        if (is_event) { W.now = t_ev; W.n_events += 1; }

        const uint32_t kind = word >> 29, aux = (word >> SLOT_BITS) & AUX_MASK;
        uint32_t slot = word & SLOT_MASK;
        uint32_t act = A_NONE;
        uint32_t node = 0, sidx = 0, rid = 0, pack = 0, edge = 0;
        bool from_box = true;
        double t0 = 0.0;
        double tm_t = 0.0; uint32_t tm_payload = 0, tm_seq = 0;
        AFL_TRACE("%s t=%.17g seq=%u kind=%u aux=%u slot=%u\n", is_item ? "it" : "ev", W.now, ev_seq, kind, aux, slot);
        const bool names_request = is_event ? (kind == K_DELIVER || kind == K_STEP_END) : (is_item && kind != I_CLIENT_LOOP && kind != I_PUT);
        if (names_request) rq_load(m, slot, t0, rid, pack);
        if (is_event) {
            if (kind == K_DELIVER) {
                conn_add(W, m, aux, -1);
                const uint32_t meta = ro(C.edges + aux).meta;
                pack += 1;
                const uint32_t tk = (meta >> 3) & 3u;
                node = tk == AF_TARGET_CLIENT ? NODE_CLIENT : (tk == AF_TARGET_LB ? NODE_LB : NODE_SERVER0 + (meta >> 5));
                if (can_fuse(W)) { act = A_NODE; from_box = false; }
                else {
                    rq_pack_set(m, slot, pack);
                    fifo_push(m, ib_word(node, IB_HEAD), ib_word(node, IB_TAIL), slot);
                    nq_push(W, m, I_PUT, node, slot);
                }
            } else if (kind == K_STEP_END) {
                sidx = aux;
                pack += (1u << 8);
                act = A_STEPS;
            } else if (kind == K_ARRIVAL) {
                rid = ++W.generated;
                slot = rq_alloc(W, m);
                W.arm_seq = W.seq++;
                W.need_arrival = 1;
                if (slot != NIL) {
                    pack = 1u; edge = (uint32_t)C.gen_edge;
                    rq_store(m, slot, W.now, rid, pack);
                    act = A_SEND;
                }
            } else if (kind == K_SPIKE) {
                double f;
                if (on_spike(W, m, f)) { tm_t = f; tm_payload = mk_payload(K_SPIKE, 0, 0); tm_seq = W.seq++; act = A_TIMER; }
            } else {
                double f;
                if (on_outage(W, m, f)) { tm_t = f; tm_payload = mk_payload(K_OUTAGE, 0, 0); tm_seq = W.seq++; act = A_TIMER; }
            }
        } else if (is_item) {
            if (kind == I_GOT) {
                node = aux;
                act = A_NODE;
            } else if (kind == I_PUT) {
                if (c32_ld(m, ib_word(aux, IB_PENDING))) {
                    c32_st(m, ib_word(aux, IB_PENDING), 0);
                    nq_push(W, m, I_GOT, aux, fifo_pop(m, ib_word(aux, IB_HEAD), ib_word(aux, IB_TAIL)));
                }
            } else if (kind == I_CLIENT_LOOP) {
                consumer_get(W, m, NODE_CLIENT);
            } else if (kind == I_RAM_OK) {
                sidx = aux;
                srv_gauge_add(W, m, sidx, SV_RAM_IN_USE, (int32_t)ep_total_ram(m, pk_ep(pack)));
                act = A_STEPS;
            } else if (kind == I_CPU_OK) {
                sidx = aux;
                if (pack & PK_WAIT) { pack &= ~PK_WAIT; srv_gauge_add(W, m, sidx, SV_READY_Q, -1); }
                pack |= PK_CORE;
                act = A_STEPS;
            } else if (kind == I_CPU_PUT) {
                sidx = aux;
                cpu_walk(W, m, sidx, NIL);
                pack &= ~PK_CORE;
                act = A_STEPS;
            } else {
                sidx = aux;
                ram_walk(W, m, sidx);
                edge = ro(C.servers + sidx).out_edge;
                act = A_SEND;
            }
        }
        AFL_SYNC();

        if (act == A_NODE) {
            act = A_NONE;
            if (node >= NODE_SERVER0) {
                sidx = node - NODE_SERVER0;
                if (from_box) consumer_get(W, m, node);
                const ServerP sp = ro(C.servers + sidx);
                pack += 1;
                uint32_t epi = 0;
                if (sp.n_ep > 1) {
                    afr::Src src = afr::make_request(C.seed, W.replica, afr::P_SERVER, rid, pk_hops(pack));
                    src.load(0);
                    epi = (uint32_t)(((uint64_t)src.w.x * sp.n_ep) >> 32);
                }
                const uint32_t ep_global = sp.ep_begin + epi;
                pack = (pack & 0xFFu) | (ep_global << 16);
                const uint32_t total_ram = ep_total_ram(m, ep_global);
                bool go = true;
                if (total_ram) {
                    if (!(can_fuse(W) && (int32_t)total_ram <= i32_ld(m, sv_word(sidx, SV_RAM_FREE)) && q_empty(W, m, sq_word(sidx, SQ_RAMQ_HEAD)))) {
                        rq_pack_set(m, slot, pack);
                        if (q_empty(W, m, sq_word(sidx, SQ_RAMQ_HEAD))) c32_st(m, sq_word(sidx, SQ_RAMQ_NEED), total_ram);
                        fifo_push(m, sq_word(sidx, SQ_RAMQ_HEAD), sq_word(sidx, SQ_RAMQ_TAIL), slot);
                        W.n_waiting += 1;
                        ram_walk(W, m, sidx);
                        go = false;
                    } else {
                        i32_st(m, sv_word(sidx, SV_RAM_FREE), i32_ld(m, sv_word(sidx, SV_RAM_FREE)) - (int32_t)total_ram);
                        srv_gauge_add(W, m, sidx, SV_RAM_IN_USE, (int32_t)total_ram);
                    }
                }
                if (go) act = A_STEPS;
            } else {
                pack += 1;
                if (node == NODE_CLIENT) {
                    if (pk_hops(pack) > 3) {
                        complete(W, m, slot, t0);
                        if (can_fuse(W)) { if (from_box) consumer_get(W, m, NODE_CLIENT); }
                        else nq_push(W, m, I_CLIENT_LOOP, 0, 0);
                    } else {
                        if (from_box) consumer_get(W, m, NODE_CLIENT);
                        edge = (uint32_t)C.client_edge;
                        act = A_SEND;
                    }
                } else {
                    const int32_t lb = C.o32_lb, n = W.lb_n;
                    if (AFL_UNLIKELY(n <= 0)) { rq_pack_set(m, slot, pack); W.flags |= AF_FLAG_LB_EMPTY; }
                    else {
                        uint32_t pick = w32_ld(m, lb);
                        if (C.lb_algo == AF_LB_ROUND_ROBIN) {
#pragma unroll 1
                            for (int32_t i = 1; i < n; ++i) w32_st(m, lb + i - 1, w32_ld(m, lb + i));
                            w32_st(m, lb + n - 1, pick);
                        } else {
                            uint32_t best = w32_ld(m, C.o32_conn + (int32_t)pick);
#pragma unroll 1
                            for (int32_t i = 1; i < n; ++i) {
                                const uint32_t e2 = w32_ld(m, lb + i), c2 = w32_ld(m, C.o32_conn + (int32_t)e2);
                                if (c2 < best) { best = c2; pick = e2; }
                            }
                        }
                        if (from_box) consumer_get(W, m, NODE_LB);
                        edge = pick;
                        act = A_SEND;
                    }
                }
            }
        }
        AFL_SYNC();

        if (act == A_STEPS) {
            act = A_NONE;
            const EndpointP ep = ro(C.endpoints + pk_ep(pack));
#pragma unroll 1
            for (;;) {
                const uint32_t st = pk_step(pack);
                if (st < ep.n_steps) {
                    const StepP sp = ro(C.steps + ep.step_begin + st);
                    if (sp.kind == AF_STEP_CPU) {
                        if (pack & PK_IO) { pack &= ~PK_IO; srv_gauge_add(W, m, sidx, SV_IO_Q, -1); }
                        if (!(pack & PK_CORE)) {
                            if (can_fuse(W) && i32_ld(m, sv_word(sidx, SV_CPU_FREE)) > 0 && q_empty(W, m, sq_word(sidx, SQ_CPUQ_HEAD))) {
                                i32_st(m, sv_word(sidx, SV_CPU_FREE), i32_ld(m, sv_word(sidx, SV_CPU_FREE)) - 1);
                                pack |= PK_CORE;
                            } else {
                                fifo_push(m, sq_word(sidx, SQ_CPUQ_HEAD), sq_word(sidx, SQ_CPUQ_TAIL), slot);
                                W.n_waiting += 1;
                                if (!cpu_walk(W, m, sidx, slot)) { pack |= PK_WAIT; srv_gauge_add(W, m, sidx, SV_READY_Q, 1); }
                                break;
                            }
                        }
                    } else {
                        if (pack & PK_CORE) {
                            i32_st(m, sv_word(sidx, SV_CPU_FREE), i32_ld(m, sv_word(sidx, SV_CPU_FREE)) + 1);
                            if (can_fuse(W)) {
                                if (AFL_UNLIKELY(!q_empty(W, m, sq_word(sidx, SQ_CPUQ_HEAD)))) cpu_walk(W, m, sidx, NIL);
                                pack &= ~PK_CORE;
                                continue;
                            }
                            nq_push(W, m, I_CPU_PUT, sidx, slot);
                            break;
                        }
                        if (!(pack & PK_IO)) { pack |= PK_IO; srv_gauge_add(W, m, sidx, SV_IO_Q, 1); }
                    }
                    const double dur = sp.c_dur >= 0 ? row_val(m, sp.c_dur) : sp.dur;
                    tm_t = W.now + dur; tm_payload = mk_payload(K_STEP_END, sidx, slot); tm_seq = W.seq++;
                    act = A_TIMER;
                    break;
                }
                if (pack & PK_CORE) {
                    i32_st(m, sv_word(sidx, SV_CPU_FREE), i32_ld(m, sv_word(sidx, SV_CPU_FREE)) + 1);
                    if (can_fuse(W)) {
                        if (AFL_UNLIKELY(!q_empty(W, m, sq_word(sidx, SQ_CPUQ_HEAD)))) cpu_walk(W, m, sidx, NIL);
                        pack &= ~PK_CORE;
                        continue;
                    }
                    nq_push(W, m, I_CPU_PUT, sidx, slot);
                    break;
                }
                if (pack & PK_IO) { pack &= ~PK_IO; srv_gauge_add(W, m, sidx, SV_IO_Q, -1); }
                const uint32_t total_ram = ep.c_ram >= 0 ? (uint32_t)row_val(m, ep.c_ram) : ep.total_ram;
                if (total_ram) {
                    srv_gauge_add(W, m, sidx, SV_RAM_IN_USE, -(int32_t)total_ram);
                    i32_st(m, sv_word(sidx, SV_RAM_FREE), i32_ld(m, sv_word(sidx, SV_RAM_FREE)) + (int32_t)total_ram);
                    if (!can_fuse(W)) { nq_push(W, m, I_RAM_PUT, sidx, slot); break; }
                    if (AFL_UNLIKELY(!q_empty(W, m, sq_word(sidx, SQ_RAMQ_HEAD)))) ram_walk(W, m, sidx);
                }
                edge = ro(C.servers + sidx).out_edge;
                act = A_SEND;
                break;
            }
            if (act != A_SEND) rq_pack_set(m, slot, pack);
        }
        AFL_SYNC();

        {
            const bool send = act == A_SEND;
            uint32_t s = 0; double dropout = 0.0, mean = 0.0, sigma = 0.0; int dist = 0;
            if (send) {
                act = A_NONE;
                const EdgeP E = ro(C.edges + edge);
                s = W.seq++;
                dropout = E.c_drop >= 0 ? row_val(m, E.c_drop) : E.dropout;
                mean = E.c_mean >= 0 ? row_val(m, E.c_mean) : E.mean;
                sigma = E.c_sigma >= 0 ? row_val(m, E.c_sigma) : E.sigma;
                dist = (int)(E.meta & 7u);
            }
            const bool fast = send && (dist == 1  || dist == 3 );
            const bool ride = !send && (is_event || is_item) && !finish && W.gap_cnt < 2u && !W.g_done
                              && W.g_vnow < W.horizon && W.g_vnow < W.g_wend && W.g_lam > 0.0;
            double u = 0.0, transit = 0.0;
            if (send && !fast) {
                const afr::EdgeDraw d = afr::edge_draw(C.seed, W.replica, rid, pk_hops(pack), dist, mean, sigma, dropout);
                u = d.u; transit = d.transit;
            }
            AFL_SYNC();
            if (fast || ride) {
                const uint32_t k0 = (uint32_t)C.seed, k1 = (uint32_t)(C.seed >> 32);
                const uint32_t tag = (afr::P_EDGE << 24) | ((pk_hops(pack) & 0xFFFFu) << 8);
                afr::U4 c;
                c.x = send ? rid : (W.g_pos >> 1); c.y = send ? tag : (afr::P_GEN << 24);
                c.z = (uint32_t)W.replica; c.w = (uint32_t)(W.replica >> 32);
                afr::U4 w = afr::philox4x32_10(c, k0, k1);
                double arg = 1.0, v1 = 0.0, q = 1.0;
                bool need = true;
                if (send) {
                    u = afr::u53(w.x, w.y);
                    if (u < dropout) need = false;
                    else if (dist == 3) arg = 1.0 - afr::u53(w.z, w.w);
                    else {
                        v1 = afr::s32(w.z); const double v2 = afr::s32(w.w);
                        q = v1 * v1 + v2 * v2;
                        uint32_t blk = 0; bool second = true;
#pragma unroll 1
                        while (!(q > 0.0 && q < 1.0)) {
                            if (second) { ++blk; c.y = tag | (blk & 0xFFu); w = afr::philox4x32_10(c, k0, k1); v1 = afr::s32(w.x); const double b = afr::s32(w.y); q = v1 * v1 + b * b; }
                            else { v1 = afr::s32(w.z); const double b = afr::s32(w.w); q = v1 * v1 + b * b; }
                            second = !second;
                        }
                        arg = q;
                    }
                } else {
                    double ug = (W.g_pos & 1u) ? afr::u53(w.z, w.w) : afr::u53(w.x, w.y);
                    if (ug < 1e-15) ug = 1e-15;
                    arg = 1.0 - ug;
                }
                double L = 0.0;
                if (need) L = afr::af_log(arg);
                const bool divide = need && !(send && dist == 3);
                double D = 0.0;
                if (divide) D = send ? afr::af_div(-2.0 * L, q) : afr::af_div(-L, W.g_lam);
                if (send) {
                    if (need) {
                        if (dist == 3) transit = mean * -L;
                        else { const double v = mean + sigma * (v1 * afr::af_sqrt(D)); transit = v > 0.0 ? v : 0.0; }
                    }
                } else if (!(W.g_vnow + D > W.horizon) && !(W.g_vnow + D >= W.g_wend)) {
                    W.g_vnow += D; W.g_pos += 1u;
                    if (W.gap_cnt == 0u) W.gap0 = D; else W.gap1 = D;
                    W.gap_cnt += 1u;
                }
            }
            if (send) {
                red_add32(g32p(m, C.gi_sent + (int32_t)edge), 1u);
                if (u < dropout) {
                    c32_st(m, C.c_drop + (int32_t)edge, c32_ld(m, C.c_drop + (int32_t)edge) + 1);
                    rq_release(W, m, slot);
                } else {
                    rq_pack_set(m, slot, pack);
                    conn_add(W, m, edge, 1);
                    double effective = transit;
                    if (C.n_spike > 0) effective = transit + f64_ld(m, C.o64_spike + (int32_t)edge);
                    else effective = transit + 0.0;
                    tm_t = W.now + effective; tm_payload = mk_payload(K_DELIVER, edge, slot); tm_seq = s;
                    act = A_TIMER;
                }
            }
        }
        AFL_SYNC();

        if (act == A_TIMER) {
            if (tm_t < W.horizon) {
                if (AFL_UNLIKELY(tm_t == W.now)) W.busy |= 1u;
                heap_push(W, m, afr::d2u(tm_t), ((uint64_t)tm_seq << 32) | tm_payload);
            }
        }
    }
}

}
```

asyncflow_b200/csrc/af_lane_host.h:

```cpp
#pragma once
#include <string>
#include <vector>
#include "af_lane.cuh"

namespace aflh {

struct Tables {
    std::vector<afl::EdgeP> edges; std::vector<afl::ServerP> servers; std::vector<afl::EndpointP> endpoints;
    std::vector<afl::StepP> steps; std::vector<afl::SpikeP> spikes; std::vector<afl::OutageP> outages;
    std::vector<int32_t> lb; std::vector<afl::ColP> cols;
    int32_t n_row = 0;
};

inline bool build_tables(const AfScenario& s, const AfSweepColumn* cols, int32_t n_cols, const int32_t* alias, Tables& t, std::string& err) {
    t = Tables();
    t.edges.resize((size_t)s.n_edges);
    for (int i = 0; i < s.n_edges; ++i) {
        const AfEdge& a = s.edges[i]; afl::EdgeP& e = t.edges[(size_t)i];
        e.mean = a.mean; e.sigma = a.sigma; e.dropout = a.dropout;
        e.meta = (uint32_t)a.dist | ((uint32_t)a.target_kind << 3) | ((uint32_t)a.target_index << 5);
        e.c_mean = e.c_sigma = e.c_drop = -1; e.pad = 0; e.pad2[0] = e.pad2[1] = 0;
    }
    t.servers.resize((size_t)s.n_servers);
    for (int i = 0; i < s.n_servers; ++i) {
        const AfServer& a = s.servers[i]; afl::ServerP& v = t.servers[(size_t)i];
        v.cpu_cores = a.cpu_cores; v.ram_mb = a.ram_mb; v.out_edge = (uint32_t)a.out_edge;
        v.ep_begin = (uint32_t)a.endpoint_begin; v.n_ep = (uint32_t)a.n_endpoints; v.c_cores = v.c_ram = -1; v.pad = 0;
    }
    t.endpoints.resize((size_t)s.n_endpoints);
    for (int i = 0; i < s.n_endpoints; ++i) {
        const AfEndpoint& a = s.endpoints[i]; afl::EndpointP& p = t.endpoints[(size_t)i];
        p.step_begin = (uint32_t)a.step_begin; p.n_steps = (uint32_t)a.n_steps; p.total_ram = (uint32_t)a.total_ram; p.c_ram = -1;
    }
    t.steps.resize((size_t)s.n_steps);
    for (int i = 0; i < s.n_steps; ++i) { t.steps[(size_t)i].dur = s.steps[i].duration; t.steps[(size_t)i].kind = (uint32_t)s.steps[i].kind; t.steps[(size_t)i].c_dur = -1; }
    t.spikes.resize((size_t)s.n_spike_marks);
    for (int i = 0; i < s.n_spike_marks; ++i) {
        afl::SpikeP& p = t.spikes[(size_t)i];
        p.fire = s.spike_marks[i].fire_time; p.delta = s.spike_marks[i].delta; p.edge = (uint32_t)s.spike_marks[i].edge; p.c_delta = -1; p.pad[0] = p.pad[1] = 0;
    }
    t.outages.resize((size_t)s.n_outage_marks);
    for (int i = 0; i < s.n_outage_marks; ++i) { t.outages[(size_t)i].fire = s.outage_marks[i].fire_time; t.outages[(size_t)i].lb_edge = s.outage_marks[i].lb_edge; t.outages[(size_t)i].down = s.outage_marks[i].down; }
    t.lb.assign(s.lb_edges, s.lb_edges + s.n_lb_edges);
    t.cols.resize((size_t)n_cols);
    int32_t n_row = 0;
    for (int32_t c = 0; c < n_cols; ++c) {
        afl::ColP& k = t.cols[(size_t)c];
        k.field = cols[c].field; k.index = cols[c].index; k.slot = -1; k.pad = 0; k.base = 0.0;
        const int32_t i = k.index;
        const int32_t shared = alias && alias[c] >= 0 ? t.cols[(size_t)alias[c]].slot : -1;
#define AFLH_SLOT() (shared >= 0 ? shared : n_row++)
        switch (k.field) {
        case AF_FIELD_USERS_MEAN: k.base = s.users_mean; break;
        case AF_FIELD_USERS_SIGMA: k.base = s.users_sigma; break;
        case AF_FIELD_RATE_PER_USER: k.base = s.rate_per_user; break;
        case AF_FIELD_SERVER_CPU_CORES: k.base = s.servers[i].cpu_cores; break;
        case AF_FIELD_SERVER_RAM_MB: k.base = s.servers[i].ram_mb; break;
        case AF_FIELD_EDGE_MEAN: k.slot = AFLH_SLOT(); k.base = s.edges[i].mean; t.edges[(size_t)i].c_mean = (int16_t)k.slot; break;
        case AF_FIELD_EDGE_SIGMA: k.slot = AFLH_SLOT(); k.base = s.edges[i].sigma; t.edges[(size_t)i].c_sigma = (int16_t)k.slot; break;
        case AF_FIELD_EDGE_DROPOUT: k.slot = AFLH_SLOT(); k.base = s.edges[i].dropout; t.edges[(size_t)i].c_drop = (int16_t)k.slot; break;
        case AF_FIELD_STEP_DURATION: k.slot = AFLH_SLOT(); k.base = s.steps[i].duration; t.steps[(size_t)i].c_dur = k.slot; break;
        case AF_FIELD_ENDPOINT_RAM: k.slot = AFLH_SLOT(); k.base = s.endpoints[i].total_ram; t.endpoints[(size_t)i].c_ram = k.slot; break;
        case AF_FIELD_SPIKE_DELTA: k.slot = AFLH_SLOT(); k.base = s.spike_marks[i].delta < 0.0 ? -s.spike_marks[i].delta : s.spike_marks[i].delta;
                                   t.spikes[(size_t)i].c_delta = k.slot; break;
        default: err = "sweep: unknown field id"; return false;
        }
#undef AFLH_SLOT
    }
    if (n_row > 32000) { err = "sweep: too many looked-up columns for the lane engine"; return false; }
    t.n_row = n_row;
    return true;
}

inline std::vector<int32_t> column_aliases(const double* values, uint64_t n_rows, int32_t n_cols) {
    std::vector<int32_t> alias((size_t)n_cols, -1);
    for (int32_t c = 1; c < n_cols; ++c)
        for (int32_t a = 0; a < c && alias[(size_t)c] < 0; ++a) {
            if (alias[(size_t)a] >= 0) continue;
            uint64_t r = 0;
            while (r < n_rows && values[r * (uint64_t)n_cols + (uint64_t)c] == values[r * (uint64_t)n_cols + (uint64_t)a]) ++r;
            if (r == n_rows) alias[(size_t)c] = a;
        }
    return alias;
}

inline int32_t pending_events_estimate(const AfScenario& s, const AfSweep* sw) {
    double users = s.users_mean, rate = s.rate_per_user, edge = 0.0, steps = 0.0;
    for (int i = 0; i < s.n_edges; ++i) if (s.edges[i].mean > edge && s.edges[i].dist != AF_DIST_LOG_NORMAL) edge = s.edges[i].mean;
    for (int e = 0; e < s.n_endpoints; ++e) {
        double d = 0.0;
        for (int k = 0; k < s.endpoints[e].n_steps; ++k) d += s.steps[s.endpoints[e].step_begin + k].duration;
        if (d > steps) steps = d;
    }
    if (sw)
        for (int c = 0; c < sw->n_columns; ++c) {
            const int f = sw->columns[c].field;
            if (f != AF_FIELD_USERS_MEAN && f != AF_FIELD_RATE_PER_USER && f != AF_FIELD_EDGE_MEAN) continue;
            double mx = 0.0;
            for (uint64_t r = 0; r < sw->n_rows; ++r) { const double v = sw->values[r * (uint64_t)sw->n_columns + (uint64_t)c]; if (v > mx) mx = v; }
            if (f == AF_FIELD_USERS_MEAN) users = mx; else if (f == AF_FIELD_RATE_PER_USER) rate = mx; else if (mx > edge) edge = mx;
        }
    const int hops = s.n_lb_edges > 0 ? 4 : 3;
    const double in_flight = users * rate * (hops * edge + steps);
    const double need = in_flight + 6.0;
    return need > 100000.0 ? 100000 : (int32_t)need;
}

constexpr int32_t LANE_EVENT_CAPACITY = 512;
constexpr int32_t LANE_REQUEST_CAPACITY = 2048;

inline int32_t fixed_lane_bytes(const AfScenario& s, const Tables& t) {
    const int32_t n_series = 3 * s.n_servers + s.n_edges;
    const int32_t fix64 = (s.n_spike_marks > 0 ? s.n_edges : 0) + t.n_row;
    const int32_t fix32 = s.n_edges + afl::SV_WORDS * s.n_servers + s.n_lb_edges + (n_series + 31) / 32;
    return 8 * fix64 + 4 * fix32;
}
constexpr int32_t MIN_DYNAMIC_BYTES = 16 * 4 + 36 * 2;
inline int32_t min_lane_bytes(const AfScenario& s, const Tables& t) { return fixed_lane_bytes(s, t) + MIN_DYNAMIC_BYTES; }

inline bool make_cfg(const AfScenario& s, const AfOptions& o, const Tables& t, int32_t lane_bytes, int32_t trace_tick_cap, int32_t lanes, afl::Cfg& C, int32_t ev_need = 0, int32_t rq_min = 2) {
    C.n_edges = s.n_edges; C.n_servers = s.n_servers; C.n_endpoints = s.n_endpoints; C.n_steps = s.n_steps;
    C.n_lb_edges = s.n_lb_edges; C.lb_algo = s.lb_algo; C.gen_edge = s.gen_edge; C.client_edge = s.client_edge;
    C.n_spike = s.n_spike_marks; C.n_outage = s.n_outage_marks;
    C.users_dist = s.users_dist; C.window_s = s.window_s; C.horizon_s = s.horizon_s; C.metrics_mask = s.metrics_mask;
    C.users_mean = s.users_mean; C.users_sigma = s.users_sigma; C.rate_per_user = s.rate_per_user; C.sample_period = s.sample_period;
    C.n_series = 3 * s.n_servers + s.n_edges;
    C.n_sweep_cols = (int32_t)t.cols.size(); C.n_row = t.n_row;
    C.collect_hist = o.collect_histogram; C.collect_thr = o.collect_throughput;
    C.trace_replicas = o.trace_replicas; C.trace_clock_cap = o.trace_clock_capacity; C.trace_tick_cap = trace_tick_cap;
    C.redo = 0;
    int32_t ev_total = o.event_capacity > 0 ? o.event_capacity : LANE_EVENT_CAPACITY;
    int32_t rq_total = o.request_capacity > 0 ? o.request_capacity : LANE_REQUEST_CAPACITY;
    if (rq_total > (int32_t)afl::SLOT_MASK) rq_total = (int32_t)afl::SLOT_MASK;
    const int32_t fix64 = (C.n_spike > 0 ? C.n_edges : 0) + C.n_row;
    C.n_dirty = (C.n_series + 31) / 32;
    const int32_t fix32 = C.n_edges + afl::SV_WORDS * C.n_servers + C.n_lb_edges + C.n_dirty;
    int32_t nq_s = 0;
    int32_t rest = lane_bytes - 8 * fix64 - 4 * fix32;
    int32_t rq_s = (rest - 16 * 4) / 36;
    if (ev_need > 0) {
        const int32_t ev_even = (rest - 20 * rq_s) / 16;
        if (rq_min < 2) rq_min = 2;
        int32_t ev_try = ev_need, ev_max = (rest - 20 * rq_min) / 16;
        if (ev_try > ev_max) ev_try = ev_max;
        if (ev_try > ev_total) ev_try = ev_total;
        if (ev_try > ev_even) {
            const int32_t rq_try = (rest - 16 * ev_try) / 20;
            if (rq_try >= 2) rq_s = rq_try;
        }
    }
    if (rq_s > rq_total) rq_s = rq_total;
    int32_t ev_s = rq_s < 0 ? 0 : (rest - 20 * rq_s) / 16;
    if (ev_s > ev_total) { ev_s = ev_total; rq_s = (rest - 16 * ev_s) / 20; if (rq_s > rq_total) rq_s = rq_total; }
    if (rq_s < (rq_total < 2 ? rq_total : 2) || ev_s < (ev_total < 4 ? ev_total : 4)) return false;
    if (ev_s == ev_total && rq_s == rq_total) {
        nq_s = (rest - 16 * ev_s - 20 * rq_s) / 8;
        if (nq_s > afl::NQ_TOTAL) nq_s = afl::NQ_TOTAL;
        if (nq_s < 0) nq_s = 0;
    }
    C.ev_s = ev_s; C.ev_total = ev_total; C.rq_s = rq_s; C.rq_total = rq_total; C.nq_s = nq_s;
    C.o128_ev = 0; C.o128_rq = ev_s; C.n128 = ev_s + rq_s;
    int32_t e = 0;
    C.o64_nq = e; e += nq_s;
    C.o64_spike = e; e += C.n_spike > 0 ? C.n_edges : 0;
    C.o64_row = e; e += C.n_row;
    C.n64 = e;
    int32_t w = 0;
    C.o32_next = w; w += rq_s;
    C.o32_conn = w; w += C.n_edges;
    C.o32_srv = w; w += afl::SV_WORDS * C.n_servers;
    C.o32_lb = w; w += C.n_lb_edges;
    C.o32_dirty = w; w += C.n_dirty;
    C.n32 = w;
    C.warp_bytes = (C.n128 * 16 + C.n64 * 8 + C.n32 * 4) * lanes;
    C.gi_ev = 0 - ev_s;
    C.gi_rq = (ev_total - ev_s) - rq_s;
    C.gn128 = (ev_total - ev_s) + (rq_total - rq_s);
    C.gi_nq = 0 - nq_s;
    C.gi_acc = afl::NQ_TOTAL - nq_s;
    C.gn64 = C.gi_acc + C.n_series;
    C.gi_next = 0 - rq_s;
    int32_t hcount = rq_total - rq_s;
    C.g32_cold = hcount;
    C.c_srvq = 0; C.c_inbox = C.c_srvq + afl::SQ_WORDS * C.n_servers; C.c_drop = C.c_inbox + afl::IB_WORDS * (C.n_servers + 2);
    hcount += C.c_drop + C.n_edges;
    C.gi_smax = hcount; hcount += C.n_series;
    C.gi_sent = hcount; hcount += C.n_edges;
    C.gn32 = hcount;
    C.gwarp_bytes = ((uint64_t)C.gn128 * 16 + (uint64_t)C.gn64 * 8 + (uint64_t)C.gn32 * 4) * (uint64_t)lanes;
    return true;
}

}
```

include/asyncflow_b200.h:

```cpp
#ifndef ASYNCFLOW_B200_H
#define ASYNCFLOW_B200_H

#include <stdint.h>

#ifdef __cplusplus
extern "C" {
#endif

#define AF_ABI_VERSION 1

typedef enum AfStatus {
    AF_OK = 0,
    AF_ERR_INVALID = -1,
    AF_ERR_CUDA = -2,
    AF_ERR_STATE = -3,
    AF_ERR_NOMEM = -4
} AfStatus;

enum { AF_DIST_POISSON = 0, AF_DIST_NORMAL = 1, AF_DIST_LOG_NORMAL = 2,
       AF_DIST_EXPONENTIAL = 3, AF_DIST_UNIFORM = 4 };
enum { AF_TARGET_CLIENT = 0, AF_TARGET_LB = 1, AF_TARGET_SERVER = 2 };
enum { AF_STEP_CPU = 0, AF_STEP_IO = 1 };
enum { AF_LB_NONE = -1, AF_LB_ROUND_ROBIN = 0, AF_LB_LEAST_CONNECTIONS = 1 };
enum { AF_METRIC_READY_QUEUE = 1, AF_METRIC_IO_SLEEP = 2, AF_METRIC_RAM_IN_USE = 4,
       AF_METRIC_EDGE_CONN = 8 };

typedef struct AfEdge {
    double mean;
    double sigma;
    double dropout;
    int32_t dist;
    int32_t target_kind;
    int32_t target_index;
    int32_t reserved;
} AfEdge;

typedef struct AfServer {
    int32_t cpu_cores;
    int32_t ram_mb;
    int32_t out_edge;
    int32_t endpoint_begin;
    int32_t n_endpoints;
    int32_t reserved;
} AfServer;

typedef struct AfEndpoint {
    int32_t step_begin;
    int32_t n_steps;
    int32_t total_ram;
    int32_t reserved;
} AfEndpoint;

typedef struct AfStep {
    double duration;
    int32_t kind;
    int32_t reserved;
} AfStep;

typedef struct AfSpikeMark {
    double fire_time;
    double delta;
    int32_t edge;
    int32_t reserved;
} AfSpikeMark;

typedef struct AfOutageMark {
    double fire_time;
    int32_t lb_edge;
    int32_t down;
} AfOutageMark;

typedef struct AfScenario {
    int32_t users_dist;
    int32_t window_s;
    double users_mean;
    double users_sigma;
    double rate_per_user;
    int32_t horizon_s;
    uint32_t metrics_mask;
    double sample_period;
    int32_t n_edges, n_servers, n_endpoints, n_steps;
    int32_t n_lb_edges;
    int32_t lb_algo;
    int32_t gen_edge;
    int32_t client_edge;
    int32_t n_spike_marks, n_outage_marks;
    const AfEdge* edges;
    const AfServer* servers;
    const AfEndpoint* endpoints;
    const AfStep* steps;
    const int32_t* lb_edges;
    const AfSpikeMark* spike_marks;
    const AfOutageMark* outage_marks;
} AfScenario;

enum {
    AF_FIELD_USERS_MEAN = 0, AF_FIELD_USERS_SIGMA = 1, AF_FIELD_RATE_PER_USER = 2,
    AF_FIELD_EDGE_MEAN = 3, AF_FIELD_EDGE_SIGMA = 4, AF_FIELD_EDGE_DROPOUT = 5,
    AF_FIELD_SERVER_CPU_CORES = 6, AF_FIELD_SERVER_RAM_MB = 7,
    AF_FIELD_STEP_DURATION = 8, AF_FIELD_ENDPOINT_RAM = 9,
    AF_FIELD_SPIKE_DELTA = 10,
    AF_FIELD_COUNT = 11
};
typedef struct AfSweepColumn { int32_t field; int32_t index; } AfSweepColumn;
typedef struct AfSweep {
    int32_t n_columns;
    int32_t reserved;
    uint64_t n_rows;
    const AfSweepColumn* columns;
    const double* values;
} AfSweep;

typedef struct AfOptions {
    int32_t event_capacity;
    int32_t request_capacity;
    int32_t warps_per_block;
    int32_t blocks_per_sm;
    int32_t collect_histogram;
    int32_t collect_throughput;
    int32_t trace_replicas;
    int32_t trace_clock_capacity;
} AfOptions;

#define AF_HIST_BINS 4096
#define AF_HIST_SUB_BITS 7
#define AF_HIST_MIN_EXP (-20)

enum { AF_FLAG_EVENT_OVERFLOW = 1, AF_FLAG_REQUEST_OVERFLOW = 2, AF_FLAG_TRACE_TRUNCATED = 4,
       AF_FLAG_NOWQ_OVERFLOW = 8,
       AF_FLAG_LB_EMPTY = 16       };

typedef struct AfReplicaStats {
    uint64_t n_events;
    uint32_t generated;
    uint32_t completed;
    uint32_t flags;
    uint32_t n_ticks;
    uint32_t peak_events;
    uint32_t peak_requests;
    double lat_sum;
    double lat_sumsq;
    double lat_min;
    double lat_max;
    double p50, p95, p99;
} AfReplicaStats;

typedef struct af_engine af_engine;

int af_abi_version(void);
int af_engine_create(int device, af_engine** out);
void af_engine_destroy(af_engine* e);
const char* af_last_error(const af_engine* e);

int af_engine_configure(af_engine* e, const AfOptions* opt);
enum { AF_MODE_AUTO = 0, AF_MODE_WARP = 1, AF_MODE_LANE = 2, AF_MODE_TWO_PASS = 3 };
int af_engine_set_mode(af_engine* e, int mode);
int af_scenario_upload(af_engine* e, const AfScenario* host_pod);
int af_sweep_upload(af_engine* e, const AfSweep* sweep, uint64_t first_replica);

int af_run(af_engine* e, uint64_t seed, uint64_t replica_begin, uint64_t replica_end);
int af_sync(af_engine* e);
int af_last_run_ms(af_engine* e, float* ms_total, float* ms_sim_kernel);
uint64_t af_launch_count(const af_engine* e);
typedef struct AfRunPasses {
    int32_t lane_pass, warp_pass;
    int32_t lane_warps_per_sm;
    int32_t lane_bytes;
    int32_t lane_events_smem, lane_requests_smem;
    uint64_t lane_replicas;
    uint64_t warp_replicas;
} AfRunPasses;
int af_last_run_passes(af_engine* e, AfRunPasses* out);

int af_fetch_stats(af_engine* e, AfReplicaStats* out, uint64_t n);
int af_fetch_edge_counts(af_engine* e, uint32_t* sent, uint32_t* dropped, uint64_t n);
int af_fetch_histograms(af_engine* e, uint32_t* out, uint64_t n);
int af_fetch_throughput(af_engine* e, uint32_t* out, uint64_t n);
int af_fetch_sampled(af_engine* e, uint64_t* sums, uint32_t* maxima, uint64_t n);
int af_reduce_histograms(af_engine* e, uint64_t* out_bins);
int af_fetch_trace_clocks(af_engine* e, uint64_t local_replica, double* start_finish,
                          uint64_t capacity_pairs, uint64_t* n_pairs);
int af_fetch_trace_series(af_engine* e, uint64_t local_replica, uint32_t* values,
                          uint64_t capacity_ticks, uint64_t* n_ticks);

enum { AF_SELFTEST_EDGE = 0, AF_SELFTEST_GEN_UNIFORM = 1, AF_SELFTEST_GEN_USERS = 2, AF_SELFTEST_ENDPOINT = 3 };
int af_selftest_rng(af_engine* e, uint64_t seed, uint64_t replica, int kind, int dist, double mean, double sigma,
                    uint32_t hop, uint64_t n, double* out_a, double* out_b);

#ifdef __cplusplus
}
#endif
#endif
```

Baseline: 642.9 million.

## Share one per-lane smem pool between event heap and request slots, split per sweep row

Replaces the fixed split of each lane's shared memory between the event heap and request table with a single 16-byte pool. Events grow from the bottom and requests from the top, and the boundary is chosen per replica from a per-row Little's-law estimate uploaded with the sweep. The shared-memory request free list becomes a 32-bit bitmask, which removes the per-slot next-pointer array from shared memory. The aim is to keep more of the hot heap and request data in shared memory for sweeps with heterogeneous load. In exchange it caps shared request slots at 32, adds per-replica state and branching, and bumps the ABI.

```diff
diff --git a/asyncflow_b200/_capi.py b/asyncflow_b200/_capi.py
--- a/asyncflow_b200/_capi.py
+++ b/asyncflow_b200/_capi.py
@@ -4,7 +4,7 @@
 import ctypes as C
 from pathlib import Path
 
-AF_ABI_VERSION = 1
+AF_ABI_VERSION = 2
 AF_HIST_BINS = 4096
 AF_HIST_SUB_BITS = 7
 AF_HIST_MIN_EXP = -20
@@ -109,7 +109,7 @@
 class AfRunPasses(C.Structure):
     _fields_ = [("lane_pass", C.c_int32), ("warp_pass", C.c_int32), ("lane_warps_per_sm", C.c_int32),
                 ("lane_bytes", C.c_int32), ("lane_events_smem", C.c_int32), ("lane_requests_smem", C.c_int32),
-                ("lane_replicas", C.c_uint64), ("warp_replicas", C.c_uint64)]
+                ("lane_replicas", C.c_uint64), ("warp_replicas", C.c_uint64), ("lane_pool_elems", C.c_int32)]
 
 
 class EngineUnavailable(RuntimeError):
diff --git a/asyncflow_b200/csrc/af_engine.cu b/asyncflow_b200/csrc/af_engine.cu
--- a/asyncflow_b200/csrc/af_engine.cu
+++ b/asyncflow_b200/csrc/af_engine.cu
@@ -216,11 +216,14 @@
     std::vector<AfSweepColumn> h_sweep_cols;
     std::vector<int32_t> h_sweep_alias;
     int32_t ev_need = 0;
-    DevBuf d_sweep_cols, d_sweep_vals;
+    std::vector<int32_t> h_row_need;
+    int32_t row_need_max = 0;
+    DevBuf d_sweep_cols, d_sweep_vals, d_row_need;
     int mode = AF_MODE_AUTO;
     aflh::Tables lt;
     DevBuf d_l_edges, d_l_servers, d_l_eps, d_l_steps, d_l_spikes, d_l_outages, d_l_lb, d_l_cols, d_gtier, d_redo_list, d_redo_count, d_counter2;
     afl::Cfg C_host{};
+    int32_t last_ev_s = 0, last_rq_s = 0;
     bool last_lane = false, last_warp = false; int last_lane_warps = 0;
     DevBuf d_sp_evt, d_sp_evk, d_sp_rq, d_sp_nx;
     DevBuf d_stats, d_sent, d_dropped, d_hist, d_thr, d_ssum, d_smax, d_tclk, d_tser, d_tcnt, d_counter, d_htot;
@@ -297,7 +300,7 @@
     DevBuf* bufs[] = {&e->d_l_edges, &e->d_l_servers, &e->d_l_eps, &e->d_l_steps, &e->d_l_spikes, &e->d_l_outages, &e->d_l_lb, &e->d_l_cols,
                       &e->d_gtier, &e->d_redo_list, &e->d_redo_count, &e->d_counter2,
                       &e->d_edges, &e->d_servers, &e->d_eps, &e->d_steps, &e->d_lb, &e->d_spikes, &e->d_outages,
-                      &e->d_sweep_cols, &e->d_sweep_vals, &e->d_sp_evt, &e->d_sp_evk, &e->d_sp_rq, &e->d_sp_nx,
+                      &e->d_sweep_cols, &e->d_sweep_vals, &e->d_row_need, &e->d_sp_evt, &e->d_sp_evk, &e->d_sp_rq, &e->d_sp_nx,
                       &e->d_stats, &e->d_sent, &e->d_dropped, &e->d_hist, &e->d_thr, &e->d_ssum, &e->d_smax,
                       &e->d_tclk, &e->d_tser, &e->d_tcnt, &e->d_counter, &e->d_htot};
     for (DevBuf* b : bufs) b->release();
@@ -343,7 +346,7 @@
     e->sc.outage_marks = e->h_outages.data();
     e->have_scenario = true;
     e->sweep_cols = 0; e->sweep_rows = 0; e->h_sweep_cols.clear();
-    e->ev_need = aflh::pending_events_estimate(e->sc, nullptr);
+    e->ev_need = aflh::pending_events_estimate(e->sc, nullptr); e->row_need_max = 0;
     e->ran = false;
     return AF_OK;
 }
@@ -353,7 +356,7 @@
     if (!e->have_scenario) return e->fail(AF_ERR_STATE, "af_sweep_upload before af_scenario_upload");
     AF_CUDA(e, cudaSetDevice(e->device), "cudaSetDevice");
     AF_CUDA(e, cudaStreamSynchronize(e->stream), "sync before sweep upload");
-    if (!sw || sw->n_columns == 0 || sw->n_rows == 0) { e->sweep_cols = 0; e->sweep_rows = 0; e->h_sweep_cols.clear(); e->ev_need = aflh::pending_events_estimate(e->sc, nullptr); return AF_OK; }
+    if (!sw || sw->n_columns == 0 || sw->n_rows == 0) { e->sweep_cols = 0; e->sweep_rows = 0; e->h_sweep_cols.clear(); e->row_need_max = 0; return AF_OK; }
     if (!sw->columns || !sw->values) return e->fail(AF_ERR_INVALID, "sweep: null columns/values");
     const AfScenario& s = e->sc;
     for (int c = 0; c < sw->n_columns; ++c) {
@@ -389,12 +392,15 @@
         }
     e->h_sweep_cols.assign(sw->columns, sw->columns + sw->n_columns);
     e->h_sweep_alias = aflh::column_aliases(sw->values, sw->n_rows, sw->n_columns);
-    e->ev_need = aflh::pending_events_estimate(e->sc, sw);
+    e->row_need_max = aflh::row_events_estimates(e->sc, *sw, e->h_row_need);
     size_t cb = (size_t)sw->n_columns * sizeof(AfSweepColumn), vb = (size_t)sw->n_columns * sw->n_rows * sizeof(double);
     AF_CUDA(e, e->d_sweep_cols.ensure(cb), "sweep columns");
     AF_CUDA(e, e->d_sweep_vals.ensure(vb), "sweep values");
+    AF_CUDA(e, e->d_row_need.ensure(sw->n_rows * sizeof(int32_t)), "sweep row estimates");
     AF_CUDA(e, cudaMemcpyAsync(e->d_sweep_cols.p, sw->columns, cb, cudaMemcpyHostToDevice, e->stream), "sweep columns H2D");
     AF_CUDA(e, cudaMemcpyAsync(e->d_sweep_vals.p, sw->values, vb, cudaMemcpyHostToDevice, e->stream), "sweep values H2D");
+    AF_CUDA(e, cudaMemcpyAsync(e->d_row_need.p, e->h_row_need.data(), sw->n_rows * sizeof(int32_t), cudaMemcpyHostToDevice, e->stream),
+            "sweep row estimates H2D");
     AF_CUDA(e, cudaStreamSynchronize(e->stream), "sweep upload");
     e->sweep_cols = sw->n_columns; e->sweep_rows = sw->n_rows; e->sweep_first = first_replica;
     return AF_OK;
@@ -448,10 +454,18 @@
     }
     if (lane) {
         memset(&C, 0, sizeof C);
-        if (!aflh::make_cfg(e->sc, o, e->lt, lane_budget(e, lane_warps), afh::trace_tick_capacity(e->sc), 32, C, getenv("ASYNCFLOW_B200_EVEN_SPLIT") ? 0 : e->ev_need,
+        const bool even = getenv("ASYNCFLOW_B200_EVEN_SPLIT") != nullptr;
+        if (!aflh::make_cfg(e->sc, o, e->lt, lane_budget(e, lane_warps), afh::trace_tick_capacity(e->sc), 32, C, even ? 0 : e->ev_need,
                             getenv("ASYNCFLOW_B200_RQ_MIN") ? atoi(getenv("ASYNCFLOW_B200_RQ_MIN")) : 2)) {
             if (e->mode == AF_MODE_LANE) return e->fail(AF_ERR_INVALID, "scenario tables do not fit a lane's shared memory (thread-per-replica engine)");
             lane = false;
+        } else {
+            const bool rows = !even && e->sweep_cols > 0;
+            const bool all_rows = rows && begin >= e->sweep_first && end - e->sweep_first <= e->sweep_rows;
+            int32_t heaviest = even ? 0 : (rows ? e->row_need_max : e->ev_need);
+            if (rows && !all_rows && e->ev_need > heaviest) heaviest = e->ev_need;
+            aflh::pool_split(C, heaviest, e->last_ev_s, e->last_rq_s);
+            if (rows) { C.need_first = e->sweep_first; C.need_rows = e->sweep_rows; }
         }
     }
     const bool warp = e->mode != AF_MODE_LANE;
@@ -548,6 +562,7 @@
         C.spikes = (const afl::SpikeP*)e->d_l_spikes.p; C.outages = (const afl::OutageP*)e->d_l_outages.p;
         C.lb_edges = (const int32_t*)e->d_l_lb.p; C.cols = (const afl::ColP*)e->d_l_cols.p;
         C.sweep_vals = G.sweep_vals; C.sweep_first = G.sweep_first; C.sweep_rows = G.sweep_rows;
+        C.row_need = C.need_rows ? (const int32_t*)e->d_row_need.p : nullptr;
         C.gtier = (unsigned char*)e->d_gtier.p;
         C.stats = G.stats; C.edge_sent = G.edge_sent; C.edge_dropped = G.edge_dropped; C.hist = G.hist; C.thr = G.thr;
         C.samp_sum = G.samp_sum; C.samp_max = G.samp_max; C.trace_clocks = G.trace_clocks; C.trace_series = G.trace_series;
@@ -636,7 +651,8 @@
     out->lane_pass = e->last_lane ? 1 : 0; out->warp_pass = e->last_warp ? 1 : 0;
     out->lane_warps_per_sm = e->last_lane_warps;
     out->lane_bytes = e->last_lane ? e->C_host.warp_bytes / 32 : 0;
-    out->lane_events_smem = e->last_lane ? e->C_host.ev_s : 0; out->lane_requests_smem = e->last_lane ? e->C_host.rq_s : 0;
+    out->lane_events_smem = e->last_lane ? e->last_ev_s : 0; out->lane_requests_smem = e->last_lane ? e->last_rq_s : 0;
+    out->lane_pool_elems = e->last_lane ? e->C_host.pool : 0;
     out->lane_replicas = e->last_lane ? e->last_n : 0;
     out->warp_replicas = e->last_warp ? e->last_n : 0;
     if (e->last_lane && e->last_warp) {
diff --git a/asyncflow_b200/csrc/af_lane.cuh b/asyncflow_b200/csrc/af_lane.cuh
--- a/asyncflow_b200/csrc/af_lane.cuh
+++ b/asyncflow_b200/csrc/af_lane.cuh
@@ -71,19 +71,21 @@
     int32_t n_series, n_sweep_cols, n_row;
     int32_t collect_hist, collect_thr, trace_replicas, trace_clock_cap, trace_tick_cap;
     int32_t redo;
-    int32_t ev_s, ev_total, rq_s, rq_total, nq_s;
-    int32_t o128_ev, o128_rq, n128;
+    int32_t ev_total, rq_total, nq_s;
+    int32_t pool, ev_lo, rq_floor, ev_s, rq_s;
+    int32_t n128;
     int32_t o64_nq, o64_spike, o64_row, n64;
-    int32_t o32_next, o32_conn, o32_srv, o32_lb, o32_dirty, n_dirty, n32;
+    int32_t o32_conn, o32_srv, o32_lb, o32_dirty, n_dirty, n32;
     int32_t warp_bytes;
-    int32_t gi_ev, gi_rq, gn128;
+    int32_t gi_rq, gn128;
     int32_t gi_nq, gi_acc, gn64;
-    int32_t gi_next, g32_cold, gi_smax, gi_sent, gn32;
+    int32_t g32_cold, gi_smax, gi_sent, gn32;
     int32_t c_srvq, c_inbox, c_drop;
     uint64_t gwarp_bytes;
     const EdgeP* edges; const ServerP* servers; const EndpointP* endpoints; const StepP* steps;
     const SpikeP* spikes; const OutageP* outages; const int32_t* lb_edges; const ColP* cols;
     const double* sweep_vals; uint64_t sweep_first, sweep_rows;
+    const int32_t* row_need; uint64_t need_first, need_rows;
     unsigned char* gtier;
     AfReplicaStats* stats; uint32_t* edge_sent; uint32_t* edge_dropped;
     uint32_t* hist; uint32_t* thr; uint64_t* samp_sum; uint32_t* samp_max;
@@ -170,13 +172,6 @@
 AFL_IN void st_t64(const Mem& m, int32_t os, int32_t gi, int32_t idx, int32_t split, uint64_t v) {
     if (AFL_LIKELY(idx < split)) sm_st64(a64(m, os + idx), v); else *g64p(m, gi + idx) = v;
 }
-AFL_IN uint32_t ld_t32(const Mem& m, int32_t os, int32_t gi, int32_t idx, int32_t split) {
-    if (AFL_LIKELY(idx < split)) return sm_ld32(a32(m, os + idx));
-    return *g32p(m, gi + idx);
-}
-AFL_IN void st_t32(const Mem& m, int32_t os, int32_t gi, int32_t idx, int32_t split, uint32_t v) {
-    if (AFL_LIKELY(idx < split)) sm_st32(a32(m, os + idx), v); else *g32p(m, gi + idx) = v;
-}
 
 struct St {
     uint64_t replica, local;
@@ -184,7 +179,9 @@
     uint32_t seq; int32_t ev_n; uint32_t peak_ev;
     uint64_t arr_t; uint32_t arr_seq, arr_on;
     uint32_t nq_head, nq_tail, busy;
-    uint32_t rq_free, rq_free_hi, rq_hw, rq_live, peak_rq;
+    int32_t ev_s, rq_s;
+    uint32_t rq_mask;
+    uint32_t rq_free_hi, rq_hw, rq_live, peak_rq;
     uint32_t n_waiting;
     double g_vnow, g_wend, g_lam;
     uint32_t g_pos, generated, g_done, need_arrival, arm_seq;
@@ -205,24 +202,41 @@
     return p.c_ram >= 0 ? (uint32_t)row_val(m, p.c_ram) : p.total_ram;
 }
 
-AFL_IN void rq_load(const Mem& m, uint32_t s, double& t0, uint32_t& rid, uint32_t& pack) {
+constexpr int32_t RQ_BITS = 32;
+AFL_IN int32_t pool_events(int32_t pool, int32_t ev_lo, int32_t rq_floor, int32_t ev_total, int32_t rq_total, int32_t need) {
+    int32_t ev = need < pool - rq_floor ? need : pool - rq_floor;
+    if (ev < ev_lo) ev = ev_lo;
+    const int32_t rq_cap = rq_total < RQ_BITS ? rq_total : RQ_BITS;
+    if (ev < pool - rq_cap) ev = pool - rq_cap;
+    return ev < ev_total ? ev : ev_total;
+}
+#if AFL_DEVICE
+AFL_IN uint32_t lowest_bit(uint32_t x) { return (uint32_t)__ffs((int)x) - 1u; }
+#else
+AFL_IN uint32_t lowest_bit(uint32_t x) { return (uint32_t)__builtin_ctz(x); }
+#endif
+
+AFL_IN uint32_t rq_sm(const Mem& m, uint32_t s) { return a128(m, AFL_C.pool - 1 - (int32_t)s); }
+AFL_IN unsigned char* rq_gl(const Mem& m, uint32_t s) { return g128p(m, AFL_C.gi_rq + (int32_t)s); }
+AFL_IN void rq_load(const St& W, const Mem& m, uint32_t s, double& t0, uint32_t& rid, uint32_t& pack) {
     uint64_t a, b;
-    ld_t128(m, AFL_C.o128_rq, AFL_C.gi_rq, (int32_t)s, AFL_C.rq_s, a, b);
+    if (AFL_LIKELY((int32_t)s < W.rq_s)) sm_ld128(rq_sm(m, s), a, b); else gl_ld128(rq_gl(m, s), a, b);
     t0 = afr::u2d(a); rid = (uint32_t)b; pack = (uint32_t)(b >> 32);
 }
-AFL_IN void rq_store(const Mem& m, uint32_t s, double t0, uint32_t rid, uint32_t pack) {
-    st_t128(m, AFL_C.o128_rq, AFL_C.gi_rq, (int32_t)s, AFL_C.rq_s, afr::d2u(t0), (uint64_t)rid | ((uint64_t)pack << 32));
-}
-AFL_IN uint32_t rq_pack(const Mem& m, uint32_t s) {
-    if (AFL_LIKELY((int32_t)s < AFL_C.rq_s)) return sm_ld32(a128(m, AFL_C.o128_rq + (int32_t)s) + 12u);
-    return *reinterpret_cast<const uint32_t*>(g128p(m, AFL_C.gi_rq + (int32_t)s) + 12);
-}
-AFL_IN void rq_pack_set(const Mem& m, uint32_t s, uint32_t v) {
-    if (AFL_LIKELY((int32_t)s < AFL_C.rq_s)) sm_st32(a128(m, AFL_C.o128_rq + (int32_t)s) + 12u, v);
-    else *reinterpret_cast<uint32_t*>(g128p(m, AFL_C.gi_rq + (int32_t)s) + 12) = v;
-}
-AFL_IN uint32_t rq_next(const Mem& m, uint32_t s) { return ld_t32(m, AFL_C.o32_next, AFL_C.gi_next, (int32_t)s, AFL_C.rq_s); }
-AFL_IN void rq_next_set(const Mem& m, uint32_t s, uint32_t v) { st_t32(m, AFL_C.o32_next, AFL_C.gi_next, (int32_t)s, AFL_C.rq_s, v); }
+AFL_IN void rq_store(const St& W, const Mem& m, uint32_t s, double t0, uint32_t rid, uint32_t pack) {
+    const uint64_t a = afr::d2u(t0), b = (uint64_t)rid | ((uint64_t)pack << 32);
+    if (AFL_LIKELY((int32_t)s < W.rq_s)) sm_st128(rq_sm(m, s), a, b); else gl_st128(rq_gl(m, s), a, b);
+}
+AFL_IN uint32_t rq_pack(const St& W, const Mem& m, uint32_t s) {
+    if (AFL_LIKELY((int32_t)s < W.rq_s)) return sm_ld32(rq_sm(m, s) + 12u);
+    return *reinterpret_cast<const uint32_t*>(rq_gl(m, s) + 12);
+}
+AFL_IN void rq_pack_set(const St& W, const Mem& m, uint32_t s, uint32_t v) {
+    if (AFL_LIKELY((int32_t)s < W.rq_s)) sm_st32(rq_sm(m, s) + 12u, v);
+    else *reinterpret_cast<uint32_t*>(rq_gl(m, s) + 12) = v;
+}
+AFL_IN uint32_t rq_next(const Mem& m, uint32_t s) { return *g32p(m, (int32_t)s); }
+AFL_IN void rq_next_set(const Mem& m, uint32_t s, uint32_t v) { *g32p(m, (int32_t)s) = v; }
 
 #if AFL_DEVICE
 __device__ __forceinline__ void red_add64(uint64_t* p, uint64_t v) { atomicAdd(reinterpret_cast<unsigned long long*>(p), (unsigned long long)v); }
@@ -239,8 +253,7 @@
 #endif
 AFL_IN uint32_t rq_alloc(St& W, const Mem& m) {
     uint32_t s;
-    if (W.rq_free != NIL) { s = W.rq_free; W.rq_free = rq_next(m, s); }
-    else if ((int32_t)W.rq_hw < AFL_C.rq_s) { s = W.rq_hw++; }
+    if (W.rq_mask != 0u) { s = lowest_bit(W.rq_mask); W.rq_mask &= W.rq_mask - 1u; }
     else if (W.rq_free_hi != NIL) { s = W.rq_free_hi; W.rq_free_hi = rq_next(m, s); }
     else if ((int32_t)W.rq_hw < AFL_C.rq_total) { s = W.rq_hw++; }
     else { W.flags |= AF_FLAG_REQUEST_OVERFLOW; return NIL; }
@@ -249,7 +262,7 @@
     return s;
 }
 AFL_IN void rq_release(St& W, const Mem& m, uint32_t s) {
-    if ((int32_t)s < AFL_C.rq_s) { rq_next_set(m, s, W.rq_free); W.rq_free = s; }
+    if ((int32_t)s < W.rq_s) W.rq_mask |= 1u << s;
     else { rq_next_set(m, s, W.rq_free_hi); W.rq_free_hi = s; }
     --W.rq_live;
 }
@@ -273,8 +286,8 @@
     return s;
 }
 
-AFL_IN void ev_get(const Mem& m, int32_t i, uint64_t& t, uint64_t& k) { ld_t128(m, AFL_C.o128_ev, AFL_C.gi_ev, i, AFL_C.ev_s, t, k); }
-AFL_IN void ev_set(const Mem& m, int32_t i, uint64_t t, uint64_t k) { st_t128(m, AFL_C.o128_ev, AFL_C.gi_ev, i, AFL_C.ev_s, t, k); }
+AFL_IN void ev_get(const St& W, const Mem& m, int32_t i, uint64_t& t, uint64_t& k) { ld_t128(m, 0, -W.ev_s, i, W.ev_s, t, k); }
+AFL_IN void ev_set(const St& W, const Mem& m, int32_t i, uint64_t t, uint64_t k) { st_t128(m, 0, -W.ev_s, i, W.ev_s, t, k); }
 AFL_IN bool ev_less(uint64_t ta, uint64_t ka, uint64_t tb, uint64_t kb) {
     return ta < tb || (ta == tb && (uint32_t)(ka >> 32) < (uint32_t)(kb >> 32));
 }
@@ -288,18 +301,18 @@
     while (i > 0) {
         const int32_t p = (i - 1) >> 2;
         uint64_t tp, kp;
-        ev_get(m, p, tp, kp);
+        ev_get(W, m, p, tp, kp);
         if (!ev_less(tb, key, tp, kp)) break;
-        ev_set(m, i, tp, kp);
+        ev_set(W, m, i, tp, kp);
         i = p;
     }
-    ev_set(m, i, tb, key);
+    ev_set(W, m, i, tb, key);
 }
 AFL_IN void heap_pop(St& W, const Mem& m) {
     const int32_t n = --W.ev_n;
     if (n == 0) return;
     uint64_t tl, kl;
-    ev_get(m, n, tl, kl);
+    ev_get(W, m, n, tl, kl);
     const int32_t last = n - 1;
     int32_t i = 0;
 #pragma unroll 1
@@ -309,21 +322,21 @@
         const int32_t c1 = c + 1 < last ? c + 1 : last, c3 = c + 3 < last ? c + 3 : last;
         int32_t c2 = c + 2 < last ? c + 2 : last;
         uint64_t t0, k0, t1, k1, t2, k2, t3, k3;
-        if (AFL_LIKELY(c3 < AFL_C.ev_s)) {
-            sm_ld128(a128(m, AFL_C.o128_ev + c), t0, k0); sm_ld128(a128(m, AFL_C.o128_ev + c1), t1, k1);
-            sm_ld128(a128(m, AFL_C.o128_ev + c2), t2, k2); sm_ld128(a128(m, AFL_C.o128_ev + c3), t3, k3);
+        if (AFL_LIKELY(c3 < W.ev_s)) {
+            sm_ld128(a128(m, c), t0, k0); sm_ld128(a128(m, c1), t1, k1);
+            sm_ld128(a128(m, c2), t2, k2); sm_ld128(a128(m, c3), t3, k3);
         } else {
-            ev_get(m, c, t0, k0); ev_get(m, c1, t1, k1); ev_get(m, c2, t2, k2); ev_get(m, c3, t3, k3);
+            ev_get(W, m, c, t0, k0); ev_get(W, m, c1, t1, k1); ev_get(W, m, c2, t2, k2); ev_get(W, m, c3, t3, k3);
         }
         int32_t b = c;
         if (ev_less(t1, k1, t0, k0)) { t0 = t1; k0 = k1; b = c1; }
         if (ev_less(t3, k3, t2, k2)) { t2 = t3; k2 = k3; c2 = c3; }
         if (ev_less(t2, k2, t0, k0)) { t0 = t2; k0 = k2; b = c2; }
         if (!ev_less(t0, k0, tl, kl)) break;
-        ev_set(m, i, t0, k0);
+        ev_set(W, m, i, t0, k0);
         i = b;
     }
-    ev_set(m, i, tl, kl);
+    ev_set(W, m, i, tl, kl);
 }
 
 AFL_IN uint64_t nq_ld(const Mem& m, uint32_t pos) {
@@ -458,7 +471,7 @@
         const uint32_t w = fifo_pop(m, sq_word(sidx, SQ_RAMQ_HEAD), sq_word(sidx, SQ_RAMQ_TAIL));
         W.n_waiting -= 1;
         const uint32_t h = c32_ld(m, sq_word(sidx, SQ_RAMQ_HEAD));
-        if (h != NIL) c32_st(m, sq_word(sidx, SQ_RAMQ_NEED), ep_total_ram(m, pk_ep(rq_pack(m, h))));
+        if (h != NIL) c32_st(m, sq_word(sidx, SQ_RAMQ_NEED), ep_total_ram(m, pk_ep(rq_pack(W, m, h))));
         i32_st(m, sv_word(sidx, SV_RAM_FREE), i32_ld(m, sv_word(sidx, SV_RAM_FREE)) - (int32_t)need);
         nq_push(W, m, I_RAM_OK, sidx, w);
     }
@@ -548,7 +561,13 @@
     W.now = 0.0; W.horizon = (double)C.horizon_s; W.seq = 0;
     W.ev_n = 0; W.peak_ev = 0; W.arr_t = 0; W.arr_seq = 0; W.arr_on = 0;
     W.nq_head = 0; W.nq_tail = 0; W.busy = 0;
-    W.rq_free = NIL; W.rq_free_hi = NIL; W.rq_hw = 0; W.rq_live = 0; W.peak_rq = 0; W.n_waiting = 0;
+    const uint64_t nr = W.replica - C.need_first;
+    if (C.row_need != nullptr && nr < C.need_rows) {
+        W.ev_s = pool_events(C.pool, C.ev_lo, C.rq_floor, C.ev_total, C.rq_total, C.row_need[nr]);
+        W.rq_s = C.pool - W.ev_s;
+    } else { W.ev_s = C.ev_s; W.rq_s = C.rq_s; }
+    W.rq_mask = W.rq_s >= RQ_BITS ? ~0u : (1u << W.rq_s) - 1u;
+    W.rq_free_hi = NIL; W.rq_hw = (uint32_t)W.rq_s; W.rq_live = 0; W.peak_rq = 0; W.n_waiting = 0;
     W.g_vnow = 0.0; W.g_wend = 0.0; W.g_lam = 0.0; W.g_pos = 0; W.generated = 0; W.g_done = 0;
     W.gap0 = 0.0; W.gap1 = 0.0; W.gap_cnt = 0;
     W.lb_n = C.n_lb_edges; W.spike_cur = 0; W.outage_cur = 0;
@@ -709,7 +728,7 @@
                 } else {
                     const bool have_heap = W.ev_n > 0, have_ev = have_heap || W.arr_on != 0;
                     uint64_t tb = 0, key = 0;
-                    if (have_heap) sm_ld128(a128(m, AFL_C.o128_ev), tb, key);
+                    if (have_heap) sm_ld128(m.s128, tb, key);
                     const uint64_t root_t = tb;
                     bool take_arr = false;
                     if (W.arr_on) {
@@ -728,7 +747,7 @@
                     if (!is_item && !finish) {
                         bool more;
                         if (take_arr) { W.arr_on = 0u; more = have_heap && root_t == tb; }
-                        else { heap_pop(W, m); more = (W.ev_n > 0 && sm_ld64(a128(m, AFL_C.o128_ev)) == tb) || (W.arr_on && W.arr_t == tb); }
+                        else { heap_pop(W, m); more = (W.ev_n > 0 && sm_ld64(m.s128) == tb) || (W.arr_on && W.arr_t == tb); }
                         W.busy = (W.busy & ~1u) | (more ? 1u : 0u);
                         t_ev = afr::u2d(tb); ev_seq = (uint32_t)(key >> 32); word = (uint32_t)key;
                         is_event = true;
@@ -755,7 +774,7 @@
         double tm_t = 0.0; uint32_t tm_payload = 0, tm_seq = 0;
         AFL_TRACE("%s t=%.17g seq=%u kind=%u aux=%u slot=%u\n", is_item ? "it" : "ev", W.now, ev_seq, kind, aux, slot);
         const bool names_request = is_event ? (kind == K_DELIVER || kind == K_STEP_END) : (is_item && kind != I_CLIENT_LOOP && kind != I_PUT);
-        if (names_request) rq_load(m, slot, t0, rid, pack);
+        if (names_request) rq_load(W, m, slot, t0, rid, pack);
         if (is_event) {
             if (kind == K_DELIVER) {
                 conn_add(W, m, aux, -1);
@@ -765,7 +784,7 @@
                 node = tk == AF_TARGET_CLIENT ? NODE_CLIENT : (tk == AF_TARGET_LB ? NODE_LB : NODE_SERVER0 + (meta >> 5));
                 if (can_fuse(W)) { act = A_NODE; from_box = false; }
                 else {
-                    rq_pack_set(m, slot, pack);
+                    rq_pack_set(W, m, slot, pack);
                     fifo_push(m, ib_word(node, IB_HEAD), ib_word(node, IB_TAIL), slot);
                     nq_push(W, m, I_PUT, node, slot);
                 }
@@ -780,7 +799,7 @@
                 W.need_arrival = 1;
                 if (slot != NIL) {
                     pack = 1u; edge = (uint32_t)C.gen_edge;
-                    rq_store(m, slot, W.now, rid, pack);
+                    rq_store(W, m, slot, W.now, rid, pack);
                     act = A_SEND;
                 }
             } else if (kind == K_SPIKE) {
@@ -843,7 +862,7 @@
                 bool go = true;
                 if (total_ram) {
                     if (!(can_fuse(W) && (int32_t)total_ram <= i32_ld(m, sv_word(sidx, SV_RAM_FREE)) && q_empty(W, m, sq_word(sidx, SQ_RAMQ_HEAD)))) {
-                        rq_pack_set(m, slot, pack);
+                        rq_pack_set(W, m, slot, pack);
                         if (q_empty(W, m, sq_word(sidx, SQ_RAMQ_HEAD))) c32_st(m, sq_word(sidx, SQ_RAMQ_NEED), total_ram);
                         fifo_push(m, sq_word(sidx, SQ_RAMQ_HEAD), sq_word(sidx, SQ_RAMQ_TAIL), slot);
                         W.n_waiting += 1;
@@ -869,7 +888,7 @@
                     }
                 } else {
                     const int32_t lb = C.o32_lb, n = W.lb_n;
-                    if (AFL_UNLIKELY(n <= 0)) { rq_pack_set(m, slot, pack); W.flags |= AF_FLAG_LB_EMPTY; }
+                    if (AFL_UNLIKELY(n <= 0)) { rq_pack_set(W, m, slot, pack); W.flags |= AF_FLAG_LB_EMPTY; }
                     else {
                         uint32_t pick = w32_ld(m, lb);
                         if (C.lb_algo == AF_LB_ROUND_ROBIN) {
@@ -954,7 +973,7 @@
                 act = A_SEND;
                 break;
             }
-            if (act != A_SEND) rq_pack_set(m, slot, pack);
+            if (act != A_SEND) rq_pack_set(W, m, slot, pack);
         }
         AFL_SYNC();
 
@@ -1031,7 +1050,7 @@
                     c32_st(m, C.c_drop + (int32_t)edge, c32_ld(m, C.c_drop + (int32_t)edge) + 1);
                     rq_release(W, m, slot);
                 } else {
-                    rq_pack_set(m, slot, pack);
+                    rq_pack_set(W, m, slot, pack);
                     conn_add(W, m, edge, 1);
                     double effective = transit;
                     if (C.n_spike > 0) effective = transit + f64_ld(m, C.o64_spike + (int32_t)edge);
diff --git a/asyncflow_b200/csrc/af_lane_host.h b/asyncflow_b200/csrc/af_lane_host.h
--- a/asyncflow_b200/csrc/af_lane_host.h
+++ b/asyncflow_b200/csrc/af_lane_host.h
@@ -84,14 +84,31 @@
     return alias;
 }
 
-inline int32_t pending_events_estimate(const AfScenario& s, const AfSweep* sw) {
-    double users = s.users_mean, rate = s.rate_per_user, edge = 0.0, steps = 0.0;
+inline int32_t littles_law_events(const AfScenario& s, double users, double rate, double edge, double steps) {
+    const int hops = s.n_lb_edges > 0 ? 4 : 3;
+    const double in_flight = users * rate * (hops * edge + steps);
+    const double need = in_flight + 6.0;
+    return need > 100000.0 ? 100000 : (int32_t)need;
+}
+inline double longest_edge(const AfScenario& s) {
+    double edge = 0.0;
     for (int i = 0; i < s.n_edges; ++i) if (s.edges[i].mean > edge && s.edges[i].dist != AF_DIST_LOG_NORMAL) edge = s.edges[i].mean;
+    return edge;
+}
+inline double longest_endpoint(const AfScenario& s, const double* dur) {
+    double steps = 0.0;
     for (int e = 0; e < s.n_endpoints; ++e) {
         double d = 0.0;
-        for (int k = 0; k < s.endpoints[e].n_steps; ++k) d += s.steps[s.endpoints[e].step_begin + k].duration;
+        for (int k = 0; k < s.endpoints[e].n_steps; ++k) d += dur[s.endpoints[e].step_begin + k];
         if (d > steps) steps = d;
     }
+    return steps;
+}
+inline int32_t pending_events_estimate(const AfScenario& s, const AfSweep* sw) {
+    double users = s.users_mean, rate = s.rate_per_user, edge = longest_edge(s);
+    std::vector<double> dur((size_t)s.n_steps);
+    for (int k = 0; k < s.n_steps; ++k) dur[(size_t)k] = s.steps[k].duration;
+    const double steps = longest_endpoint(s, dur.data());
     if (sw)
         for (int c = 0; c < sw->n_columns; ++c) {
             const int f = sw->columns[c].field;
@@ -100,10 +117,39 @@
             for (uint64_t r = 0; r < sw->n_rows; ++r) { const double v = sw->values[r * (uint64_t)sw->n_columns + (uint64_t)c]; if (v > mx) mx = v; }
             if (f == AF_FIELD_USERS_MEAN) users = mx; else if (f == AF_FIELD_RATE_PER_USER) rate = mx; else if (mx > edge) edge = mx;
         }
-    const int hops = s.n_lb_edges > 0 ? 4 : 3;
-    const double in_flight = users * rate * (hops * edge + steps);
-    const double need = in_flight + 6.0;
-    return need > 100000.0 ? 100000 : (int32_t)need;
+    return littles_law_events(s, users, rate, edge, steps);
+}
+inline int32_t row_events_estimates(const AfScenario& s, const AfSweep& sw, std::vector<int32_t>& out) {
+    out.assign((size_t)sw.n_rows, 0);
+    std::vector<double> mean((size_t)s.n_edges), dur((size_t)s.n_steps);
+    bool per_row_steps = false;
+    for (int c = 0; c < sw.n_columns; ++c) per_row_steps = per_row_steps || sw.columns[c].field == AF_FIELD_STEP_DURATION;
+    for (int k = 0; k < s.n_steps; ++k) dur[(size_t)k] = s.steps[k].duration;
+    double steps = longest_endpoint(s, dur.data());
+    int32_t mx = 0;
+    for (uint64_t r = 0; r < sw.n_rows; ++r) {
+        const double* row = sw.values + r * (uint64_t)sw.n_columns;
+        double users = s.users_mean, rate = s.rate_per_user;
+        for (int i = 0; i < s.n_edges; ++i) mean[(size_t)i] = s.edges[i].mean;
+        if (per_row_steps) for (int k = 0; k < s.n_steps; ++k) dur[(size_t)k] = s.steps[k].duration;
+        for (int c = 0; c < sw.n_columns; ++c) {
+            const int i = sw.columns[c].index;
+            switch (sw.columns[c].field) {
+            case AF_FIELD_USERS_MEAN: users = row[c]; break;
+            case AF_FIELD_RATE_PER_USER: rate = row[c]; break;
+            case AF_FIELD_EDGE_MEAN: mean[(size_t)i] = row[c]; break;
+            case AF_FIELD_STEP_DURATION: dur[(size_t)i] = row[c]; break;
+            default: break;
+            }
+        }
+        double edge = 0.0;
+        for (int i = 0; i < s.n_edges; ++i) if (mean[(size_t)i] > edge && s.edges[i].dist != AF_DIST_LOG_NORMAL) edge = mean[(size_t)i];
+        if (per_row_steps) steps = longest_endpoint(s, dur.data());
+        const int32_t need = littles_law_events(s, users, rate, edge, steps);
+        out[(size_t)r] = need;
+        if (need > mx) mx = need;
+    }
+    return mx;
 }
 
 constexpr int32_t LANE_EVENT_CAPACITY = 512;
@@ -117,6 +163,11 @@
 }
 constexpr int32_t MIN_DYNAMIC_BYTES = 16 * 4 + 36 * 2;
 inline int32_t min_lane_bytes(const AfScenario& s, const Tables& t) { return fixed_lane_bytes(s, t) + MIN_DYNAMIC_BYTES; }
+
+inline void pool_split(const afl::Cfg& C, int32_t need, int32_t& ev_s, int32_t& rq_s) {
+    ev_s = afl::pool_events(C.pool, C.ev_lo, C.rq_floor, C.ev_total, C.rq_total, need);
+    rq_s = C.pool - ev_s;
+}
 
 inline bool make_cfg(const AfScenario& s, const AfOptions& o, const Tables& t, int32_t lane_bytes, int32_t trace_tick_cap, int32_t lanes, afl::Cfg& C, int32_t ev_need = 0, int32_t rq_min = 2) {
     C.n_edges = s.n_edges; C.n_servers = s.n_servers; C.n_endpoints = s.n_endpoints; C.n_steps = s.n_steps;
@@ -136,51 +187,38 @@
     C.n_dirty = (C.n_series + 31) / 32;
     const int32_t fix32 = C.n_edges + afl::SV_WORDS * C.n_servers + C.n_lb_edges + C.n_dirty;
     int32_t nq_s = 0;
-    int32_t rest = lane_bytes - 8 * fix64 - 4 * fix32;
-    int32_t rq_s = (rest - 16 * 4) / 36;
-    if (ev_need > 0) {
-        const int32_t ev_even = (rest - 20 * rq_s) / 16;
-        if (rq_min < 2) rq_min = 2;
-        int32_t ev_try = ev_need, ev_max = (rest - 20 * rq_min) / 16;
-        if (ev_try > ev_max) ev_try = ev_max;
-        if (ev_try > ev_total) ev_try = ev_total;
-        if (ev_try > ev_even) {
-            const int32_t rq_try = (rest - 16 * ev_try) / 20;
-            if (rq_try >= 2) rq_s = rq_try;
-        }
-    }
-    if (rq_s > rq_total) rq_s = rq_total;
-    int32_t ev_s = rq_s < 0 ? 0 : (rest - 20 * rq_s) / 16;
-    if (ev_s > ev_total) { ev_s = ev_total; rq_s = (rest - 16 * ev_s) / 20; if (rq_s > rq_total) rq_s = rq_total; }
-    if (rq_s < (rq_total < 2 ? rq_total : 2) || ev_s < (ev_total < 4 ? ev_total : 4)) return false;
-    if (ev_s == ev_total && rq_s == rq_total) {
-        nq_s = (rest - 16 * ev_s - 20 * rq_s) / 8;
+    const int32_t rest = lane_bytes - 8 * fix64 - 4 * fix32;
+    const int32_t rq_cap = rq_total < afl::RQ_BITS ? rq_total : afl::RQ_BITS;
+    int32_t pool = rest < 0 ? 0 : rest / 16;
+    if (pool > ev_total + rq_cap) {
+        pool = ev_total + rq_cap;
+        nq_s = (rest - 16 * pool) / 8;
         if (nq_s > afl::NQ_TOTAL) nq_s = afl::NQ_TOTAL;
-        if (nq_s < 0) nq_s = 0;
-    }
-    C.ev_s = ev_s; C.ev_total = ev_total; C.rq_s = rq_s; C.rq_total = rq_total; C.nq_s = nq_s;
-    C.o128_ev = 0; C.o128_rq = ev_s; C.n128 = ev_s + rq_s;
+    }
+    if (pool < (ev_total < 4 ? ev_total : 4) + (rq_total < 2 ? rq_total : 2)) return false;
+    C.pool = pool; C.ev_lo = pool - (pool - 4) / 2; C.rq_floor = rq_min < 2 ? 2 : rq_min;
+    C.row_need = nullptr; C.need_first = 0; C.need_rows = 0;
+    C.ev_total = ev_total; C.rq_total = rq_total; C.nq_s = nq_s;
+    pool_split(C, ev_need, C.ev_s, C.rq_s);
+    C.n128 = pool;
     int32_t e = 0;
     C.o64_nq = e; e += nq_s;
     C.o64_spike = e; e += C.n_spike > 0 ? C.n_edges : 0;
     C.o64_row = e; e += C.n_row;
     C.n64 = e;
     int32_t w = 0;
-    C.o32_next = w; w += rq_s;
     C.o32_conn = w; w += C.n_edges;
     C.o32_srv = w; w += afl::SV_WORDS * C.n_servers;
     C.o32_lb = w; w += C.n_lb_edges;
     C.o32_dirty = w; w += C.n_dirty;
     C.n32 = w;
     C.warp_bytes = (C.n128 * 16 + C.n64 * 8 + C.n32 * 4) * lanes;
-    C.gi_ev = 0 - ev_s;
-    C.gi_rq = (ev_total - ev_s) - rq_s;
-    C.gn128 = (ev_total - ev_s) + (rq_total - rq_s);
+    C.gi_rq = ev_total - pool;
+    C.gn128 = ev_total + rq_total - pool;
     C.gi_nq = 0 - nq_s;
     C.gi_acc = afl::NQ_TOTAL - nq_s;
     C.gn64 = C.gi_acc + C.n_series;
-    C.gi_next = 0 - rq_s;
-    int32_t hcount = rq_total - rq_s;
+    int32_t hcount = rq_total;
     C.g32_cold = hcount;
     C.c_srvq = 0; C.c_inbox = C.c_srvq + afl::SQ_WORDS * C.n_servers; C.c_drop = C.c_inbox + afl::IB_WORDS * (C.n_servers + 2);
     hcount += C.c_drop + C.n_edges;
diff --git a/include/asyncflow_b200.h b/include/asyncflow_b200.h
--- a/include/asyncflow_b200.h
+++ b/include/asyncflow_b200.h
@@ -7,7 +7,7 @@
 extern "C" {
 #endif
 
-#define AF_ABI_VERSION 1
+#define AF_ABI_VERSION 2
 
 typedef enum AfStatus {
     AF_OK = 0,
@@ -169,6 +169,7 @@
     int32_t lane_events_smem, lane_requests_smem;
     uint64_t lane_replicas;
     uint64_t warp_replicas;
+    int32_t lane_pool_elems;
 } AfRunPasses;
 int af_last_run_passes(af_engine* e, AfRunPasses* out);
 
```

Measured after the change: 698.2 million (median of 6 runs). 8.6% higher.
